# LarissaReames-NOAA/MPASSIT

Measured on AMD Instinct MI355X. Metric: interpolated 3-D fields/sec (nCells x nLev -> nx x ny), higher is better.
Workload: dtype f64

## Files before the change

### mpassit_amd/csrc/k_prims.hip

```cpp
#include "mpg_internal.h"

#define SCAN_NT 256
#define SCAN_IPT 16
#define SCAN_TILE (SCAN_NT * SCAN_IPT)

__global__ __launch_bounds__(SCAN_NT) void k_scan_block_sums(const int32_t *__restrict__ in, int64_t n, int32_t *__restrict__ bsum) {
  __shared__ int32_t ws[SCAN_NT / 64];
  const int64_t base = (int64_t)blockIdx.x * SCAN_TILE;
  int32_t v = 0;
#pragma unroll
  for (int k = 0; k < SCAN_IPT; ++k) {
    const int64_t i = base + (int64_t)k * SCAN_NT + threadIdx.x;
    if (i < n) v += in[i];
  }
  for (int o = 32; o > 0; o >>= 1) v += __shfl_down(v, o);
  if ((threadIdx.x & 63) == 0) ws[threadIdx.x >> 6] = v;
  __syncthreads();
  if (threadIdx.x == 0) bsum[blockIdx.x] = ws[0] + ws[1] + ws[2] + ws[3];
}

__device__ __forceinline__ int32_t block_excl_scan(int32_t v, int32_t *total) {
  __shared__ int32_t ws[SCAN_NT / 64 + 1];
  const int lane = threadIdx.x & 63, w = threadIdx.x >> 6;
  int32_t inc = v;
  for (int o = 1; o < 64; o <<= 1) {
    const int32_t t = __shfl_up(inc, o);
    if (lane >= o) inc += t;
  }
  __syncthreads();
  if (lane == 63) ws[w] = inc;
  __syncthreads();
  int32_t off = 0;
  for (int k = 0; k < w; ++k) off += ws[k];
  *total = ws[0] + ws[1] + ws[2] + ws[3];
  return off + inc - v;
}

__global__ __launch_bounds__(SCAN_NT) void k_scan_sums(int32_t *__restrict__ bsum, int64_t nb) {
  int32_t carry = 0;
  for (int64_t b0 = 0; b0 < nb; b0 += SCAN_NT) {
    const int64_t i = b0 + threadIdx.x;
    const int32_t v = i < nb ? bsum[i] : 0;
    int32_t total;
    const int32_t ex = block_excl_scan(v, &total);
    if (i < nb) bsum[i] = carry + ex;
    carry += total;
  }
}

__global__ __launch_bounds__(SCAN_NT) void k_scan_apply(const int32_t *in, int64_t n, const int32_t *__restrict__ boff, int32_t *out) {
  const int64_t base = (int64_t)blockIdx.x * SCAN_TILE + (int64_t)threadIdx.x * SCAN_IPT;
  int32_t v[SCAN_IPT];
  int32_t sum = 0;
#pragma unroll
  for (int k = 0; k < SCAN_IPT; ++k) {
    v[k] = base + k < n ? in[base + k] : 0;
    sum += v[k];
  }
  int32_t total;
  int32_t run = boff[blockIdx.x] + block_excl_scan(sum, &total);
#pragma unroll
  for (int k = 0; k < SCAN_IPT; ++k) {
    if (base + k < n) out[base + k] = run;
    run += v[k];
  }
}

int mpg_scan_excl_i32(const int32_t *in, int32_t *out, int64_t n, hipStream_t s) {
  if (n <= 0) return MPG_SUCCESS;
  const int64_t nb = (n + SCAN_TILE - 1) / SCAN_TILE;
  TmpBuf<int32_t> bsum;
  int rc;
  if ((rc = bsum.alloc((size_t)nb, s))) return rc;
  k_scan_block_sums<<<(unsigned)nb, SCAN_NT, 0, s>>>(in, n, bsum.p);
  k_scan_sums<<<1, SCAN_NT, 0, s>>>(bsum.p, nb);
  k_scan_apply<<<(unsigned)nb, SCAN_NT, 0, s>>>(in, n, bsum.p, out);
  MPG_HIP(hipGetLastError());
  return MPG_SUCCESS;
}

__global__ __launch_bounds__(256) void k_sum_i32_i64(const int32_t *__restrict__ in, int64_t n, unsigned long long *__restrict__ out) {
  __shared__ long long ws[4];
  long long v = 0;
  for (int64_t i = blockIdx.x * (int64_t)blockDim.x + threadIdx.x; i < n; i += (int64_t)gridDim.x * blockDim.x) v += in[i];
  for (int o = 32; o > 0; o >>= 1) v += __shfl_down(v, o);
  if ((threadIdx.x & 63) == 0) ws[threadIdx.x >> 6] = v;
  __syncthreads();
  if (threadIdx.x == 0) atomicAdd(out, (unsigned long long)(ws[0] + ws[1] + ws[2] + ws[3]));
}

int mpg_sum_i32_i64(const int32_t *in, int64_t n, long long *out_dev, hipStream_t s) {
  MPG_HIP(hipMemsetAsync(out_dev, 0, sizeof(long long), s));
  if (n > 0) k_sum_i32_i64<<<(unsigned)std::min<int64_t>((n + 255) / 256, 1024), 256, 0, s>>>(in, n, (unsigned long long *)out_dev);
  MPG_HIP(hipGetLastError());
  return MPG_SUCCESS;
}

const void *mpg_anchor_k_prims() { return (const void *)k_scan_apply; }
```

### mpassit_amd/csrc/k_store_conserve.hip

```cpp
#include <cstring>


#pragma clang fp contract(off)

#include "geom.h"
#include "mpg_internal.h"
#include "conserve_clip.h"

#define CONS_BUF (CONS_MAXV + 4)
#define CONS_STACK 64
static_assert(CONS_STACK >= WalkCap<PyrTree>::FILTER, "the stack holds the walk's proven bound (tree_walk.h): its guard is never taken");
#define CONS_QUEUE 2048

#define CAND_CAP 24
#define CONS_SPILL 256
#define CONS_BIGBOX 128
#define CONS_COOP_NT 64
template <int MODE>
__global__ __launch_bounds__(MODE == 3 ? 128 : CONS_COOP_NT) void k_conserve_raster(int64_t nCells, int maxEdges, const int32_t *__restrict__ voc,
                                                         const double *__restrict__ vx, const double *__restrict__ vy,
                                                         const double *__restrict__ vz, PyramidView pyr, int nx, int ny,
                                                         const double *__restrict__ qx, const double *__restrict__ qy,
                                                         const double *__restrict__ qz, const double *__restrict__ qarea,
                                                         const double *__restrict__ qsph, int32_t *__restrict__ cnt_src,
                                                         int32_t *__restrict__ tmp_dst, int32_t *__restrict__ ovf, int32_t *__restrict__ n_ovf,
                                                         uint8_t *__restrict__ flip, const int32_t *__restrict__ poff,
                                                         int32_t *__restrict__ pair_c, int32_t *__restrict__ pair_p, const float *__restrict__ vij,
                                                         float pad_coef, float pad_latlon, float e_max, int32_t *__restrict__ spill, int spill_cap) {
  constexpr bool COOP = MODE == 5 || MODE == 6;
  int64_t c = COOP ? (int64_t)ovf[blockIdx.x] : MODE == 7 ? (int64_t)pair_c[blockIdx.x] : blockIdx.x * (int64_t)blockDim.x + threadIdx.x;
  if (c >= nCells) return;
  if (MODE == 5 && cnt_src[c] != CAND_CAP + 1) return;
  if (MODE == 5 && n_ovf && threadIdx.x == 0) atomicAdd(n_ovf + 3, 1);
  if (spill && (int)blockIdx.x >= spill_cap && COOP) spill = nullptr;
  if (MODE == 6 && spill) {
    const int n = poff[c + 1] - poff[c];
    if (n <= CONS_SPILL) {
      if (n_ovf && threadIdx.x == 0) atomicAdd(n_ovf + 4, 1);
      for (int k = threadIdx.x; k < n; k += blockDim.x) {
        pair_c[poff[c] + k] = (int32_t)c;
        pair_p[poff[c] + k] = spill[(int64_t)blockIdx.x * CONS_SPILL + k];
      }
      return;
    }
  }
  int found = 0;
  dv3 poly[CONS_MAXV];
  int n = 0;
  for (int j = 0; j < maxEdges && n < CONS_MAXV; ++j) {
    int32_t v = voc[c * maxEdges + j];
    if (v > 0) poly[n++] = dv3{vx[v - 1], vy[v - 1], vz[v - 1]};
  }
  if (n < 3) return;
  double area = 0.0;
  for (int i = 1; i + 1 < n; ++i) area += sph_tri_area(poly[0], poly[i], poly[i + 1]);
  if (area == 0.0) return;
  if (MODE == 3 && flip) flip[c] = area < 0.0;
  if (area < 0.0)
    for (int i = 0; i < n / 2; ++i) {
      dv3 t = poly[i]; poly[i] = poly[n - 1 - i]; poly[n - 1 - i] = t;
    }
  double lo[3] = {2, 2, 2}, hi[3] = {-2, -2, -2}, e2 = 0.0;
  for (int i = 0; i < n; ++i) {
    lo[0] = fmin(lo[0], poly[i].x); hi[0] = fmax(hi[0], poly[i].x);
    lo[1] = fmin(lo[1], poly[i].y); hi[1] = fmax(hi[1], poly[i].y);
    lo[2] = fmin(lo[2], poly[i].z); hi[2] = fmax(hi[2], poly[i].z);
    dv3 d = poly[i] - poly[0];
    e2 = fmax(e2, dot3(d, d));
  }
  double pad = 2.0 * e2 + 1e-9;
#pragma unroll
  for (int k = 0; k < 3; ++k) { lo[k] -= pad; hi[k] += pad; }

  int nxc = nx + 1;
  auto candidate = [&](int i, int j) -> bool {
    const int64_t pc = (int64_t)j * nx + i;
    {
      const double4 sph = *reinterpret_cast<const double4 *>(qsph + 4 * pc);
      double sx = sph.x, sy = sph.y, sz = sph.z, r2 = sph.w;
      double ddx = fmax(fmax(lo[0] - sx, sx - hi[0]), 0.0), ddy = fmax(fmax(lo[1] - sy, sy - hi[1]), 0.0),
             ddz = fmax(fmax(lo[2] - sz, sz - hi[2]), 0.0);
      if (ddx * ddx + ddy * ddy + ddz * ddz > r2) return false;
    }
    int64_t k00 = (int64_t)j * nxc + i;
    dv3 q[4] = {dv3{qx[k00], qy[k00], qz[k00]}, dv3{qx[k00 + 1], qy[k00 + 1], qz[k00 + 1]},
                dv3{qx[k00 + nxc + 1], qy[k00 + nxc + 1], qz[k00 + nxc + 1]}, dv3{qx[k00 + nxc], qy[k00 + nxc], qz[k00 + nxc]}};
    double ql[3] = {2, 2, 2}, qh[3] = {-2, -2, -2}, qe2 = 0.0;
#pragma unroll
    for (int k = 0; k < 4; ++k) {
      ql[0] = fmin(ql[0], q[k].x); qh[0] = fmax(qh[0], q[k].x);
      ql[1] = fmin(ql[1], q[k].y); qh[1] = fmax(qh[1], q[k].y);
      ql[2] = fmin(ql[2], q[k].z); qh[2] = fmax(qh[2], q[k].z);
      dv3 d = q[k] - q[0];
      qe2 = fmax(qe2, dot3(d, d));
    }
    double qp = 2.0 * qe2 + 1e-9;
    if (ql[0] - qp > hi[0] || qh[0] + qp < lo[0] || ql[1] - qp > hi[1] || qh[1] + qp < lo[1] || ql[2] - qp > hi[2] || qh[2] + qp < lo[2]) return false;
    return fabs(qarea[pc]) > 0.0;
  };
  if ((MODE == 3 || MODE == 7) && vij) {
    float imin = 1e30f, imax = -1e30f, jmin = 1e30f, jmax = -1e30f;
    bool ok = true;
    for (int j = 0, k = 0; j < maxEdges && k < CONS_MAXV; ++j) {
      int32_t v = voc[c * maxEdges + j];
      if (v <= 0) continue;
      ++k;
      const float vi = vij[2 * (int64_t)(v - 1)], vj = vij[2 * (int64_t)(v - 1) + 1];
      ok = ok && vi == vi && vj == vj;
      imin = fminf(imin, vi); imax = fmaxf(imax, vi);
      jmin = fminf(jmin, vj); jmax = fmaxf(jmax, vj);
    }
    const float E = fmaxf(imax - imin, jmax - jmin);
    if (!ok) {
      const double *bx = pyr.box + 6 * pyr.off[pyr.nlev - 1];
      if (bx[0] > hi[0] || bx[3] < lo[0] || bx[1] > hi[1] || bx[4] < lo[1] || bx[2] > hi[2] || bx[5] < lo[2]) {
        cnt_src[c] = 0;
        return;
      }
      cnt_src[c] = CAND_CAP + 1;
      ovf[atomicAdd(n_ovf, 1)] = (int32_t)c;
      return;
    }
    if (E <= e_max) {
      const float pad = mpg_box_pad(E, pad_coef, pad_latlon, fmax(fabs(lo[2]), fabs(hi[2])));
      const int i0 = max((int)ceilf(imin - pad - 0.5f), 0), i1 = min((int)floorf(imax + pad + 0.5f), nx - 1);
      const int j0 = max((int)ceilf(jmin - pad - 0.5f), 0), j1 = min((int)floorf(jmax + pad + 0.5f), ny - 1);
      const int bw = max(i1 - i0 + 1, 0), bh = max(j1 - j0 + 1, 0);
      if (MODE == 3 && pair_c && bw * bh > CONS_BIGBOX) {
        const int qs = atomicAdd(n_ovf + 2, 1);
        if (qs < spill_cap) {
          pair_c[qs] = (int32_t)c;
          cnt_src[c] = CAND_CAP + 1;
          return;
        }
      }
      if (MODE == 7) {
        const int lane = (int)threadIdx.x, total = bw * bh;
        int slot = -1;
        bool complete = true;
        for (int base = 0; base < total && complete; base += 64) {
          const int q = base + lane;
          bool is = false;
          int32_t pc = 0;
          if (q < total) {
            const int i = i0 + q % bw, j = j0 + q / bw;
            is = candidate(i, j);
            pc = (int32_t)((int64_t)j * nx + i);
          }
          const unsigned long long mask = __ballot(is);
          const int nnew = __popcll(mask);
          if (nnew == 0) continue;
          const int pos = found + __popcll(mask & ((1ull << lane) - 1ull));
          if (found + nnew > CAND_CAP && slot < 0) {
            int sl = 0;
            if (lane == 0) {
              sl = atomicAdd(n_ovf, 1);
              ovf[sl] = (int32_t)c;
            }
            slot = __shfl(sl, 0);
            if (spill && slot < spill_cap) {
              __threadfence_block();
              for (int k = lane; k < min(found, CAND_CAP); k += 64) spill[(int64_t)slot * CONS_SPILL + k] = tmp_dst[c * CAND_CAP + k];
            } else {
              complete = false;
            }
          }
          if (is) {
            if (pos < CAND_CAP) tmp_dst[c * CAND_CAP + pos] = pc;
            if (slot >= 0 && complete && pos < CONS_SPILL) spill[(int64_t)slot * CONS_SPILL + pos] = pc;
          }
          found += nnew;
          if (slot >= 0 && found > CONS_SPILL) complete = false;
        }
        if (lane == 0) cnt_src[c] = (slot < 0 || complete) ? found : CAND_CAP + 1;
        return;
      }
      int slot = -1;
      bool complete = true;
      for (int j = j0; j <= j1; ++j)
        for (int i = i0; i <= i1; ++i) {
          if (!candidate(i, j)) continue;
          const int32_t pc = (int32_t)((int64_t)j * nx + i);
          if (found < CAND_CAP) {
            tmp_dst[c * CAND_CAP + found] = pc;
          } else {
            if (slot < 0) {
              slot = atomicAdd(n_ovf, 1);
              ovf[slot] = (int32_t)c;
              if (spill && slot < spill_cap)
                for (int k = 0; k < CAND_CAP; ++k) spill[(int64_t)slot * CONS_SPILL + k] = tmp_dst[c * CAND_CAP + k];
              else
                complete = false;
            }
            if (complete && found < CONS_SPILL) spill[(int64_t)slot * CONS_SPILL + found] = pc;
            else complete = false;
          }
          ++found;
          if (!complete) {
            j = j1;
            break;
          }
        }
      cnt_src[c] = (slot < 0 || complete) ? found : CAND_CAP + 1;
      return;
    }
  }
  if (MODE == 7) return;
  int stack[CONS_STACK];
  __shared__ int q_nodes[2][CONS_QUEUE];
  __shared__ int q_n[2], q_over, s_found;
  int seed_lev = pyr.nlev - 1, nseed = 1, cur = 0;
  if (COOP) {
    if (threadIdx.x == 0) { q_nodes[0][0] = 0; q_n[0] = 1; q_over = 0; s_found = 0; }
    __syncthreads();
    while (seed_lev > 1) {
      const int nq = q_n[cur];
      if (threadIdx.x == 0) q_n[cur ^ 1] = 0;
      __syncthreads();
      const int cnx = pyr.nx[seed_lev - 1], cny = pyr.ny[seed_lev - 1], pnx = pyr.nx[seed_lev];
      for (int k = threadIdx.x; k < nq; k += blockDim.x) {
        int node = q_nodes[cur][k], bi = node % pnx, bj = node / pnx;
        for (int ch = 0; ch < 4; ++ch) {
          int ci = 2 * bi + (ch & 1), cj = 2 * bj + (ch >> 1);
          if (ci >= cnx || cj >= cny) continue;
          const double *bx = pyr.box + 6 * (pyr.off[seed_lev - 1] + cj * cnx + ci);
          if (bx[0] > hi[0] || bx[3] < lo[0] || bx[1] > hi[1] || bx[4] < lo[1] || bx[2] > hi[2] || bx[5] < lo[2]) continue;
          int slot = atomicAdd(&q_n[cur ^ 1], 1);
          if (slot < CONS_QUEUE) q_nodes[cur ^ 1][slot] = cj * cnx + ci;
          else q_over = 1;
        }
      }
      __syncthreads();
      if (q_over) break;
      cur ^= 1;
      --seed_lev;
      __syncthreads();
    }
    nseed = q_n[cur];
  }
  for (int sk = COOP ? (int)threadIdx.x : 0; sk < nseed; sk += COOP ? (int)blockDim.x : 1) {
  const int seed = COOP ? q_nodes[cur][sk] : 0;
  int sp = 0;
  auto meets = [&](int lev_, int node_) -> bool {
    const double *bx = pyr.box + 6 * (pyr.off[lev_] + node_);
    return !(bx[0] > hi[0] || bx[3] < lo[0] || bx[1] > hi[1] || bx[4] < lo[1] || bx[2] > hi[2] || bx[5] < lo[2]);
  };
  int cur = (COOP || meets(seed_lev, seed)) ? ((seed_lev << 26) | seed) : -1;
  for (;;) {
    if (cur < 0) {
      if (sp == 0) break;
      cur = stack[--sp];
    }
    const int e = cur;
    cur = -1;
    int lev = e >> 26, node = e & ((1 << 26) - 1);
    int nxl = pyr.nx[lev];
    int bi = node % nxl, bj = node / nxl;
    if (lev == 0) {
      int i0 = bi * MPG_PYR_B0, j0 = bj * MPG_PYR_B0;
      int i1 = min(i0 + MPG_PYR_B0, nx), j1 = min(j0 + MPG_PYR_B0, ny);
      for (int j = j0; j < j1; ++j)
        for (int i = i0; i < i1; ++i) {
          if (!candidate(i, j)) continue;
          const int64_t p = (int64_t)j * nx + i;
          if (MODE == 3) {
            if (found == CAND_CAP) {
              cnt_src[c] = CAND_CAP + 1;
              ovf[atomicAdd(n_ovf, 1)] = (int32_t)c;
              return;
            }
            tmp_dst[c * CAND_CAP + found] = (int32_t)p;
            ++found;
          } else if (MODE == 5) {
            const int slot = atomicAdd(&s_found, 1);
            if (spill && slot < CONS_SPILL) spill[(int64_t)blockIdx.x * CONS_SPILL + slot] = (int32_t)p;
          } else {
            const int slot = atomicAdd(&s_found, 1);
            pair_c[poff[c] + slot] = (int32_t)c;
            pair_p[poff[c] + slot] = (int32_t)p;
          }
        }
    } else {
      int cnx = pyr.nx[lev - 1], cny = pyr.ny[lev - 1];
      bool go[4];
#pragma unroll
      for (int ch = 0; ch < 4; ++ch) {
        int ci = 2 * bi + (ch & 1), cj = 2 * bj + (ch >> 1);
        go[ch] = ci < cnx && cj < cny && meets(lev - 1, cj * cnx + ci);
      }
#pragma unroll
      for (int ch = 0; ch < 4; ++ch)
        if (go[ch]) {
          const int child = ((lev - 1) << 26) | ((2 * bj + (ch >> 1)) * cnx + 2 * bi + (ch & 1));
          if (cur < 0) cur = child;
          else if (sp < CONS_STACK) stack[sp++] = child;
        }
    }
  }
  }
  if (MODE == 3) cnt_src[c] = found;
  if (MODE == 5) {
    __syncthreads();
    if (threadIdx.x == 0) cnt_src[c] = s_found;
  }
}

__global__ __launch_bounds__(256) void k_cell_areas(int nx, int ny, const double *__restrict__ qx, const double *__restrict__ qy,
                                                    const double *__restrict__ qz, double *__restrict__ qarea,
                                                    double *__restrict__ qsph ) {
  int64_t p = blockIdx.x * (int64_t)blockDim.x + threadIdx.x;
  if (p >= (int64_t)nx * ny) return;
  int i = (int)(p % nx), j = (int)(p / nx), nxc = nx + 1;
  int64_t k00 = (int64_t)j * nxc + i;
  dv3 q0 = dv3{qx[k00], qy[k00], qz[k00]}, q1 = dv3{qx[k00 + 1], qy[k00 + 1], qz[k00 + 1]},
      q2 = dv3{qx[k00 + nxc + 1], qy[k00 + nxc + 1], qz[k00 + nxc + 1]}, q3 = dv3{qx[k00 + nxc], qy[k00 + nxc], qz[k00 + nxc]};
  qarea[p] = sph_tri_area(q0, q1, q2) + sph_tri_area(q0, q2, q3);
  dv3 cen = (q0 + q1) + (q2 + q3);
  double nn = sqrt(dot3(cen, cen));
  cen = nn > 0.0 ? cen * (1.0 / nn) : q0;
  double r2 = 0.0;
  dv3 d = q0 - cen; r2 = fmax(r2, dot3(d, d));
  d = q1 - cen; r2 = fmax(r2, dot3(d, d));
  d = q2 - cen; r2 = fmax(r2, dot3(d, d));
  d = q3 - cen; r2 = fmax(r2, dot3(d, d));
  *reinterpret_cast<double4 *>(qsph + 4 * p) = double4{cen.x, cen.y, cen.z, r2 * (1.0 + 1e-9) + 1e-18};
}

__global__ __launch_bounds__(256) void k_max_valence(int64_t nCells, int maxEdges, const int32_t *__restrict__ voc, int32_t *__restrict__ out) {
  __shared__ int smax;
  if (threadIdx.x == 0) smax = 0;
  __syncthreads();
  int mx = 0;
  for (int64_t c = blockIdx.x * (int64_t)blockDim.x + threadIdx.x; c < nCells; c += (int64_t)gridDim.x * blockDim.x) {
    int n = 0;
    for (int j = 0; j < maxEdges; ++j) n += voc[c * maxEdges + j] > 0;
    mx = max(mx, n);
  }
  atomicMax(&smax, mx);
  __syncthreads();
  if (threadIdx.x == 0) atomicMax(out, smax);
}

int mpg_k_mesh_max_valence(mpg_mesh_s *m, hipStream_t s) {
  if (m->max_valence >= 0) return MPG_SUCCESS;
  int rc;
  TmpBuf<int32_t> mv;
  if ((rc = mv.alloc(1, s))) return rc;
  MPG_HIP(hipMemsetAsync(mv.p, 0, sizeof(int32_t), s));
  const int64_t nC = m->cwn;
  int32_t hv = 0;
  if (nC > 0) k_max_valence<<<(unsigned)std::min<int64_t>((nC + 255) / 256, 2048), 256, 0, s>>>(nC, m->maxEdges, m->voc.p, mv.p);
  MPG_HIP(hipGetLastError());
  MPG_HIP(hipMemcpyAsync(&hv, mv.p, sizeof(int32_t), hipMemcpyDeviceToHost, s));
  MPG_HIP(hipStreamSynchronize(s));
  m->max_valence = hv;
  return MPG_SUCCESS;
}

__global__ __launch_bounds__(256) void k_csr_sort_rows(int64_t P, const int32_t *__restrict__ rowptr, int32_t *__restrict__ col,
                                                       double *__restrict__ val) {
  int64_t p = blockIdx.x * (int64_t)blockDim.x + threadIdx.x;
  if (p >= P) return;
  int b = rowptr[p], e = rowptr[p + 1];
  for (int i = b + 1; i < e; ++i) {
    int32_t kc = col[i];
    double kv = val[i];
    int j = i - 1;
    while (j >= b && col[j] > kc) {
      col[j + 1] = col[j];
      val[j + 1] = val[j];
      --j;
    }
    col[j + 1] = kc;
    val[j + 1] = kv;
  }
}

__global__ __launch_bounds__(256) void k_conserve_clamp_counts(int64_t nCells, const int32_t *__restrict__ cnt_src, int32_t *__restrict__ npair) {
  int64_t c = blockIdx.x * (int64_t)blockDim.x + threadIdx.x;
  if (c > nCells) return;
  int n = c < nCells ? cnt_src[c] : 0;
  npair[c] = n;
}
__global__ __launch_bounds__(256) void k_conserve_fill_pairs(int64_t nCells, const int32_t *__restrict__ npair, const int32_t *__restrict__ poff,
                                                             const int32_t *__restrict__ tmp_dst, int32_t *__restrict__ pair_c,
                                                             int32_t *__restrict__ pair_p) {
  int64_t c = blockIdx.x * (int64_t)blockDim.x + threadIdx.x;
  if (c >= nCells) return;
  const int n = npair[c], o = poff[c];
  if (n > CAND_CAP) return;
  for (int e = 0; e < n; ++e) {
    pair_c[o + e] = (int32_t)c;
    pair_p[o + e] = tmp_dst[c * CAND_CAP + e];
  }
}

template <bool RAW>
__global__ __launch_bounds__(CLIP_NT) void k_conserve_clip_pairs(int64_t npairs, const int32_t *__restrict__ pair_c, const int32_t *__restrict__ pair_p,
                                                                 int maxEdges, const int32_t *__restrict__ voc, const double *__restrict__ vx,
                                                                 const double *__restrict__ vy, const double *__restrict__ vz,
                                                                 const uint8_t *__restrict__ flip, int nx, const double *__restrict__ qx,
                                                                 const double *__restrict__ qy, const double *__restrict__ qz,
                                                                 const double *__restrict__ qarea, int cb, double *__restrict__ pair_val,
                                                                 int32_t *__restrict__ count, int32_t *__restrict__ truncated) {
  extern __shared__ double clip_lds[];
  const int64_t t = blockIdx.x * (int64_t)CLIP_NT + threadIdx.x;
  if (t >= npairs) return;
  const LdsPoly L{clip_lds + threadIdx.x, cb};
  const int64_t c = pair_c[t], p = pair_p[t];
  int32_t vid[CONS_MAXV];
#pragma unroll
  for (int k = 0; k < CONS_MAXV; ++k) vid[k] = k < maxEdges ? voc[c * maxEdges + k] : 0;
  const bool rev = flip[c] != 0;
  int ntot = 0, vsafe = 0;
#pragma unroll
  for (int k = 0; k < CONS_MAXV; ++k) {
    if (vid[k] > 0) {
      ++ntot;
      if (vsafe == 0) vsafe = vid[k];
    }
  }
  int n = 0;
  if (vsafe > 0) {
    dv3 vc[CONS_MAXV];
#pragma unroll
    for (int k = 0; k < CONS_MAXV; ++k) {
      const int64_t v = (vid[k] > 0 ? vid[k] : vsafe) - 1;
      vc[k] = dv3{vx[v], vy[v], vz[v]};
    }
#pragma unroll
    for (int k = 0; k < CONS_MAXV; ++k)
      if (vid[k] > 0) {
        L.set(0, rev ? ntot - 1 - n : n, vc[k]);
        ++n;
      }
  }
  const int i = (int)(p % nx), j = (int)(p / nx), nxc = nx + 1;
  const int64_t k00 = (int64_t)j * nxc + i;
  dv3 q[4] = {dv3{qx[k00], qy[k00], qz[k00]}, dv3{qx[k00 + 1], qy[k00 + 1], qz[k00 + 1]},
              dv3{qx[k00 + nxc + 1], qy[k00 + nxc + 1], qz[k00 + nxc + 1]}, dv3{qx[k00 + nxc], qy[k00 + nxc], qz[k00 + nxc]}};
  double aq = qarea[p];
  if (aq < 0.0) { dv3 tq = q[1]; q[1] = q[3]; q[3] = tq; aq = -aq; }
  double ar = 0.0;
  int trunc = 0;
  if (aq > 0.0) {
    const int cur = 0;
    for (int e = 0; e < 4 && n >= 3; ++e) {
      const dv3 qa = e == 0 ? q[0] : e == 1 ? q[1] : e == 2 ? q[2] : q[3];
      const dv3 qb = e == 0 ? q[1] : e == 1 ? q[2] : e == 2 ? q[3] : q[0];
      dv3 side = qb - qa;
      if (dot3(side, side) < 1e-24) continue;
      n = clip_halfspace_lds(n, L, cross3(qa, side), cb, &trunc);
    }
    if (n >= 3) {
      double sa = 0.0;
      const dv3 v0 = L.get(cur, 0);
      for (int k = 1; k + 1 < n; ++k) sa += sph_tri_area(v0, L.get(cur, k), L.get(cur, k + 1));
      ar = sa > 0.0 ? sa : 0.0;
    }
  }
  if constexpr (RAW) {
    pair_val[t] = ar;
  } else {
    double ratio = 0.0;
    if (ar > 1e-14 * aq) {
      ratio = ar / aq;
      atomicAdd(&count[p], 1);
    }
    pair_val[t] = ratio;
  }
  if (trunc) atomicOr(truncated, 1);
}
__global__ __launch_bounds__(256) void k_conserve_scatter_pairs(int64_t npairs, const int32_t *__restrict__ pair_c, const int32_t *__restrict__ pair_p,
                                                                const double *__restrict__ pair_val, const int32_t *__restrict__ rowptr,
                                                                int32_t *__restrict__ cursor, int32_t *__restrict__ col, double *__restrict__ val,
                                                                int32_t cell0) {
  int64_t t = blockIdx.x * (int64_t)blockDim.x + threadIdx.x;
  if (t >= npairs) return;
  const double r = pair_val[t];
  if (!(r > 0.0)) return;
  const int32_t p = pair_p[t];
  const int slot = atomicAdd(&cursor[p], 1);
  col[rowptr[p] + slot] = pair_c[t] + cell0;
  val[rowptr[p] + slot] = r;
}

struct ConsPairs {
  TmpBuf<int32_t> count, cnt_src, tmp_dst, ovf, n_ovf, npair, poff, pair_c, pair_p, spill, bigq, truncated;
  TmpBuf<double> qarea, qsph, pair_val;
  TmpBuf<uint8_t> flip;
  TmpBuf<float> vij;
  int32_t npairs = 0, novf = 0, nbig = 0;
  int cb = 0;
};
static int conserve_pairs(mpg_mesh_s *m, mpg_grid_s *g, mpg_handle_s *h, hipStream_t s, bool raw, ConsPairs &X) {
  int rc;
  PointSet &cor = g->pts[MPG_STAGGERLOC_CORNER];
  const int nx = g->nx, ny = g->ny;
  const int64_t P = (int64_t)nx * ny;
  TmpBuf<int32_t> &count = X.count, &cnt_src = X.cnt_src, &tmp_dst = X.tmp_dst, &ovf = X.ovf, &n_ovf = X.n_ovf, &npair = X.npair, &poff = X.poff,
                  &pair_c = X.pair_c, &pair_p = X.pair_p;
  TmpBuf<double> &qarea = X.qarea, &qsph = X.qsph, &pair_val = X.pair_val;
  TmpBuf<uint8_t> &flip = X.flip;
  const int64_t nC = m->cwn;
  const double *vx = m->vx_g(), *vy = m->vy_g(), *vz = m->vz_g();
  if ((!raw && (rc = count.alloc((size_t)P + 1, s))) || (rc = qarea.alloc((size_t)P, s)) || (rc = qsph.alloc(4 * (size_t)P, s)) ||
      (rc = cnt_src.alloc((size_t)nC, s)) || (rc = tmp_dst.alloc((size_t)nC * CAND_CAP, s)) || (rc = ovf.alloc((size_t)nC, s)) || (rc = n_ovf.alloc(5, s)) ||
      (rc = npair.alloc((size_t)nC + 1, s)) || (rc = poff.alloc((size_t)nC + 1, s)) || (rc = flip.alloc((size_t)nC, s)))
    return rc;
  MPG_HIP(hipMemsetAsync(n_ovf.p, 0, 5 * sizeof(int32_t), s));
  MPG_HIP(hipMemsetAsync(cnt_src.p, 0, sizeof(int32_t) * (size_t)nC, s));
  MPG_HIP(hipMemsetAsync(flip.p, 0, (size_t)nC, s));
  if (!raw) MPG_HIP(hipMemsetAsync(count.p, 0, sizeof(int32_t) * (P + 1), s));
  unsigned nb = (unsigned)((nC + 127) / 128);
  PyramidView pv = mpg_pyr_view(g->cellpyr);
  TmpBuf<float> &vij = X.vij;
  const float *vijp = nullptr;
  if (mpg_grid_has_inverse(g, MPG_STAGGERLOC_CORNER) && mpg_store_boxes() && m->vwn > 0) {
    if ((rc = vij.alloc(2 * (size_t)m->vwn, s))) return rc;
    if ((rc = mpg_k_points_ij(g, m->vwn, m->vert.x.p, m->vert.y.p, m->vert.z.p, vij.p, s))) return rc;
    vijp = vij.p - 2 * m->vw0;
    h->store_path = 1;
  }
  k_cell_areas<<<(unsigned)((P + 255) / 256), 256, 0, s>>>(nx, ny, cor.x.p, cor.y.p, cor.z.p, qarea.p, qsph.p);
  const int spill_cap = (int)std::min<int64_t>(nC, 1 << 16);
  TmpBuf<int32_t> &spill = X.spill, &bigq = X.bigq;
  if ((rc = spill.alloc((size_t)spill_cap * CONS_SPILL, s)) || (rc = bigq.alloc((size_t)spill_cap, s))) return rc;
  k_conserve_raster<3><<<nb, 128, 0, s>>>(nC, m->maxEdges, m->voc.p, vx, vy, vz, pv, nx, ny, cor.x.p, cor.y.p, cor.z.p,
                                        qarea.p, qsph.p, cnt_src.p, tmp_dst.p, ovf.p, n_ovf.p, flip.p, nullptr, vijp ? bigq.p : nullptr, nullptr, vijp,
                                        (float)mpg_grid_box_pad_coef(g), (float)mpg_grid_box_pad_latlon(g), (float)mpg_grid_box_emax(g), spill.p, spill_cap);
  if (m->max_valence < 0) k_max_valence<<<(unsigned)std::min<int64_t>((nC + 255) / 256, 2048), 256, 0, s>>>(nC, m->maxEdges, m->voc.p, n_ovf.p + 1);
  MPG_HIP(hipGetLastError());
  int32_t &novf = X.novf, hv[3] = {0, 0, 0};
  MPG_HIP(hipMemcpyAsync(hv, n_ovf.p, 3 * sizeof(int32_t), hipMemcpyDeviceToHost, s));
  MPG_HIP(hipStreamSynchronize(s));
  novf = hv[0];
  if (m->max_valence < 0) m->max_valence = hv[1];
  if (hv[2] > 0) {
    k_conserve_raster<7><<<(unsigned)std::min(hv[2], spill_cap), 64, 0, s>>>(nC, m->maxEdges, m->voc.p, vx, vy, vz, pv, nx, ny, cor.x.p, cor.y.p, cor.z.p,
                                                                            qarea.p, qsph.p, cnt_src.p, tmp_dst.p, ovf.p, n_ovf.p, nullptr, nullptr, bigq.p, nullptr,
                                                                            vijp, (float)mpg_grid_box_pad_coef(g), (float)mpg_grid_box_pad_latlon(g),
                                                                            (float)mpg_grid_box_emax(g), spill.p, spill_cap);
    MPG_HIP(hipGetLastError());
    MPG_HIP(hipMemcpyAsync(&novf, n_ovf.p, sizeof(int32_t), hipMemcpyDeviceToHost, s));
    MPG_HIP(hipStreamSynchronize(s));
  }
  const unsigned coop_nt = CONS_COOP_NT;
  if (novf > 0)
    k_conserve_raster<5><<<(unsigned)novf, coop_nt, 0, s>>>(nC, m->maxEdges, m->voc.p, vx, vy, vz, pv, nx, ny, cor.x.p,
                                                       cor.y.p, cor.z.p, qarea.p, qsph.p, cnt_src.p, nullptr, ovf.p, n_ovf.p, nullptr, nullptr,
                                                       nullptr, nullptr, nullptr, 0.f, 0.f, 0.f, spill.p, spill_cap);
  k_conserve_clamp_counts<<<(unsigned)((nC + 256) / 256), 256, 0, s>>>(nC, cnt_src.p, npair.p);
  if ((rc = mpg_scan_excl_i32(npair.p, poff.p, nC + 1, s))) return rc;
  int32_t &npairs = X.npairs;
  long long total = 0;
  {
    TmpBuf<long long> tot;
    if ((rc = tot.alloc(1, s))) return rc;
    if ((rc = mpg_sum_i32_i64(npair.p, nC, tot.p, s))) return rc;
    MPG_HIP(hipMemcpyAsync(&npairs, poff.p + nC, sizeof(int32_t), hipMemcpyDeviceToHost, s));
    MPG_HIP(hipMemcpyAsync(&total, tot.p, sizeof(total), hipMemcpyDeviceToHost, s));
    MPG_HIP(hipStreamSynchronize(s));
    if (npairs < 0 || total != (long long)npairs) {
      mpg_set_error("conservative RegridStore: %lld candidate pairs exceed 2^31", total);
      return MPG_ERR_OVERFLOW;
    }
  }
  if ((rc = pair_c.alloc((size_t)npairs + 1, s)) || (rc = pair_p.alloc((size_t)npairs + 1, s)) || (rc = pair_val.alloc((size_t)npairs + 1, s))) return rc;
  k_conserve_fill_pairs<<<(unsigned)((nC + 255) / 256), 256, 0, s>>>(nC, npair.p, poff.p, tmp_dst.p, pair_c.p, pair_p.p);
  if (novf > 0)
    k_conserve_raster<6><<<(unsigned)novf, coop_nt, 0, s>>>(nC, m->maxEdges, m->voc.p, vx, vy, vz, pv, nx, ny, cor.x.p,
                                                       cor.y.p, cor.z.p, qarea.p, qsph.p, nullptr, nullptr, ovf.p, n_ovf.p, nullptr, poff.p,
                                                       pair_c.p, pair_p.p, nullptr, 0.f, 0.f, 0.f, spill.p, spill_cap);
  MPG_HIP(hipGetLastError());
  const int nv = std::max(3, std::min(m->max_valence, m->maxEdges));
  const int cb = X.cb = nv + 4 < CONS_BUF ? nv + 4 : CONS_BUF;
  const size_t clip_lds_bytes = sizeof(double) * cb * 3 * CLIP_NT;
  auto clip = raw ? k_conserve_clip_pairs<true> : k_conserve_clip_pairs<false>;
  if (clip_lds_bytes > 48 * 1024) MPG_HIP(hipFuncSetAttribute((const void *)clip, hipFuncAttributeMaxDynamicSharedMemorySize, (int)clip_lds_bytes));
  TmpBuf<int32_t> &truncated = X.truncated;
  if ((rc = truncated.alloc(1, s))) return rc;
  MPG_HIP(hipMemsetAsync(truncated.p, 0, sizeof(int32_t), s));
  if (npairs > 0)
    clip<<<(unsigned)(((int64_t)npairs + CLIP_NT - 1) / CLIP_NT), CLIP_NT, clip_lds_bytes, s>>>(
        npairs, pair_c.p, pair_p.p, m->maxEdges, m->voc.p, vx, vy, vz, flip.p, nx, cor.x.p, cor.y.p, cor.z.p, qarea.p, cb,
        pair_val.p, raw ? nullptr : count.p, truncated.p);
  MPG_HIP(hipGetLastError());
  X.nbig = std::min(hv[2], spill_cap);
  return MPG_SUCCESS;
}

int mpg_k_store_conserve(mpg_mesh_s *m, mpg_grid_s *g, mpg_handle_s *h, hipStream_t s) {
  int rc;
  PointSet &cor = g->pts[MPG_STAGGERLOC_CORNER];
  int nx = g->nx, ny = g->ny;
  int64_t P = (int64_t)nx * ny;
  if (cor.n != (int64_t)(nx + 1) * (ny + 1)) {
    mpg_set_error("conservative RegridStore needs CORNER-stagger coordinates on the destination grid");
    return MPG_ERR_INVALID_ARG;
  }
  if (m->maxEdges > CONS_MAXV) {
    mpg_set_error("conservative RegridStore: maxEdges %d > %d", m->maxEdges, CONS_MAXV);
    return MPG_ERR_UNSUPPORTED;
  }
  if (!g->cellpyr.built && (rc = mpg_k_build_cell_pyramid(cor, nx, ny, g->cellpyr, s))) return rc;
  if ((rc = mpg_walk_check<PyrTree>((int64_t)g->cellpyr.nx[0] * g->cellpyr.ny[0], "conservative RegridStore"))) return rc;
  h->kind = MPG_KIND_CSR;
  h->nnz_per_row = 0;
  h->n_src = m->nCells;
  h->n_dst = P;
  h->nx_dst = nx;
  h->ny_dst = ny;
  const int64_t nC = m->cwn;
  if (nC == 0) {
    if ((rc = h->rowptr.alloc((size_t)P + 1)) || (rc = h->col.alloc(1)) || (rc = h->val.alloc(1))) return rc;
    MPG_HIP(hipMemsetAsync(h->rowptr.p, 0, sizeof(int32_t) * (P + 1), s));
    MPG_HIP(hipStreamSynchronize(s));
    h->nnz = 0;
    return MPG_SUCCESS;
  }
  ConsPairs X;
  if ((rc = h->rowptr.alloc((size_t)P + 1)) || (rc = conserve_pairs(m, g, h, s, false, X))) return rc;
  TmpBuf<int32_t> &count = X.count, &n_ovf = X.n_ovf, &truncated = X.truncated, &pair_c = X.pair_c, &pair_p = X.pair_p;
  TmpBuf<double> &pair_val = X.pair_val;
  const int32_t npairs = X.npairs, novf = X.novf;
  const int cb = X.cb;
  if ((rc = mpg_scan_excl_i32(count.p, h->rowptr.p, P + 1, s))) return rc;
  int32_t nnz = 0, was_truncated = 0, hs[5] = {0, 0, 0, 0, 0};
  MPG_HIP(hipMemcpyAsync(hs, n_ovf.p, sizeof(hs), hipMemcpyDeviceToHost, s));
  MPG_HIP(hipMemcpyAsync(&nnz, h->rowptr.p + P, sizeof(int32_t), hipMemcpyDeviceToHost, s));
  MPG_HIP(hipMemcpyAsync(&was_truncated, truncated.p, sizeof(int32_t), hipMemcpyDeviceToHost, s));
  MPG_HIP(hipStreamSynchronize(s));
  if (was_truncated) {
    mpg_set_error("conservative RegridStore: a clipped polygon outgrew its %d vertex slots (a non-convex source cell?)", cb);
    return MPG_ERR_OVERFLOW;
  }
  if (nnz < 0) {
    mpg_set_error("conservative weight matrix exceeds 2^31 entries");
    return MPG_ERR_OVERFLOW;
  }
  h->nnz = nnz;
  h->store_stats[1] = npairs; h->store_stats[2] = novf; h->store_stats[3] = X.nbig; h->store_stats[4] = hs[3];
  h->store_stats[5] = hs[4]; h->store_stats[6] = cb;
  if ((rc = h->col.alloc((size_t)nnz + 1)) || (rc = h->val.alloc((size_t)nnz + 1))) return rc;
  MPG_HIP(hipMemsetAsync(count.p, 0, sizeof(int32_t) * (P + 1), s));
  if (npairs > 0)
    k_conserve_scatter_pairs<<<(unsigned)(((int64_t)npairs + 255) / 256), 256, 0, s>>>(npairs, pair_c.p, pair_p.p, pair_val.p, h->rowptr.p, count.p,
                                                                                      h->col.p, h->val.p, (int32_t)m->cw0);
  k_csr_sort_rows<<<(unsigned)((P + 255) / 256), 256, 0, s>>>(P, h->rowptr.p, h->col.p, h->val.p);
  MPG_HIP(hipGetLastError());
  MPG_HIP(hipStreamSynchronize(s));
  return MPG_SUCCESS;
}

__global__ __launch_bounds__(256) void k_conserve_tm_count(int64_t nCells, int maxEdges, const int32_t *__restrict__ voc, const double *__restrict__ vx,
                                                           const double *__restrict__ vy, const double *__restrict__ vz,
                                                           const int32_t *__restrict__ poff, const double *__restrict__ pair_val,
                                                           double *__restrict__ carea, int32_t *__restrict__ cnt) {
  const int64_t c = blockIdx.x * (int64_t)blockDim.x + threadIdx.x;
  if (c > nCells) return;
  if (c == nCells) {
    cnt[c] = 0;
    return;
  }
  const double a = cell_fan_area(c, maxEdges, voc, vx, vy, vz);
  carea[c] = a;
  int n = 0;
  if (a > 0.0)
    for (int t = poff[c]; t < poff[c + 1]; ++t) n += pair_val[t] > 1e-14 * a;
  cnt[c] = n;
}
__global__ __launch_bounds__(256) void k_conserve_tm_rows(int64_t nCells, const int32_t *__restrict__ poff, const int32_t *__restrict__ pair_p,
                                                          const double *__restrict__ pair_val, const double *__restrict__ carea,
                                                          const int32_t *__restrict__ rowptr, int norm_type, int32_t *__restrict__ col,
                                                          double *__restrict__ val, double *__restrict__ frac) {
  const int64_t c = blockIdx.x * (int64_t)blockDim.x + threadIdx.x;
  if (c >= nCells) return;
  const double a = carea[c];
  const int b = rowptr[c], e = rowptr[c + 1];
  if (e == b) {
    frac[c] = 0.0;
    return;
  }
  int n = 0;
  for (int t = poff[c]; t < poff[c + 1]; ++t) {
    const double I = pair_val[t];
    if (!(I > 1e-14 * a)) continue;
    const int32_t g = pair_p[t];
    int j = b + n - 1;
    while (j >= b && col[j] > g) {
      col[j + 1] = col[j];
      val[j + 1] = val[j];
      --j;
    }
    col[j + 1] = g;
    val[j + 1] = I;
    ++n;
  }
  double sum = 0.0;
  for (int q = b; q < e; ++q) sum += val[q];
  frac[c] = sum / a;
  const double d = norm_type == MPG_NORM_FRACAREA ? sum : a;
  for (int q = b; q < e; ++q) val[q] = val[q] / d;
}

int mpg_k_conserve_rows(mpg_mesh_s *m, const int32_t *poff, const int32_t *pair_col, const double *pair_val, const int32_t *truncated, int cb,
                        int norm_type, const char *who, mpg_handle_s *h, hipStream_t s, const int32_t *extra_dev, int32_t *extra_host, int nextra) {
  int rc;
  const int64_t nC = m->nCells;
  TmpBuf<double> carea;
  TmpBuf<int32_t> cnt;
  if ((rc = carea.alloc((size_t)nC, s)) || (rc = cnt.alloc((size_t)nC + 1, s))) return rc;
  const double *vx = m->vx_g(), *vy = m->vy_g(), *vz = m->vz_g();
  k_conserve_tm_count<<<(unsigned)((nC + 256) / 256), 256, 0, s>>>(nC, m->maxEdges, m->voc.p, vx, vy, vz, poff, pair_val, carea.p, cnt.p);
  MPG_HIP(hipGetLastError());
  if ((rc = mpg_scan_excl_i32(cnt.p, h->rowptr.p, nC + 1, s))) return rc;
  int32_t nnz = 0, was_truncated = 0;
  if (nextra > 0) MPG_HIP(hipMemcpyAsync(extra_host, extra_dev, sizeof(int32_t) * (size_t)nextra, hipMemcpyDeviceToHost, s));
  MPG_HIP(hipMemcpyAsync(&nnz, h->rowptr.p + nC, sizeof(int32_t), hipMemcpyDeviceToHost, s));
  MPG_HIP(hipMemcpyAsync(&was_truncated, truncated, sizeof(int32_t), hipMemcpyDeviceToHost, s));
  MPG_HIP(hipStreamSynchronize(s));
  if (was_truncated) {
    mpg_set_error("%s: a clipped polygon outgrew its %d vertex slots (a non-convex mesh cell?)", who, cb);
    return MPG_ERR_OVERFLOW;
  }
  if (nnz < 0) {
    mpg_set_error("%s: the weight matrix exceeds 2^31 entries", who);
    return MPG_ERR_OVERFLOW;
  }
  h->nnz = nnz;
  if ((rc = h->col.alloc((size_t)nnz + 1)) || (rc = h->val.alloc((size_t)nnz + 1))) return rc;
  k_conserve_tm_rows<<<(unsigned)((nC + 255) / 256), 256, 0, s>>>(nC, poff, pair_col, pair_val, carea.p, h->rowptr.p, norm_type, h->col.p, h->val.p,
                                                                  h->dst_frac.p);
  MPG_HIP(hipGetLastError());
  MPG_HIP(hipStreamSynchronize(s));
  return MPG_SUCCESS;
}

int mpg_k_store_conserve_to_mesh(mpg_grid_s *g, mpg_mesh_s *m, int norm_type, mpg_handle_s *h, hipStream_t s) {
  int rc;
  PointSet &cor = g->pts[MPG_STAGGERLOC_CORNER];
  const int nx = g->nx, ny = g->ny;
  if (cor.n != (int64_t)(nx + 1) * (ny + 1)) {
    mpg_set_error("mpg_regrid_store_conserve_to_mesh: a conservative Store needs CORNER-stagger coordinates on the source grid");
    return MPG_ERR_INVALID_ARG;
  }
  if (m->maxEdges > CONS_MAXV) {
    mpg_set_error("mpg_regrid_store_conserve_to_mesh: maxEdges %d > %d", m->maxEdges, CONS_MAXV);
    return MPG_ERR_UNSUPPORTED;
  }
  if (!g->cellpyr.built && (rc = mpg_k_build_cell_pyramid(cor, nx, ny, g->cellpyr, s))) return rc;
  if ((rc = mpg_walk_check<PyrTree>((int64_t)g->cellpyr.nx[0] * g->cellpyr.ny[0], "mpg_regrid_store_conserve_to_mesh"))) return rc;
  const int64_t nC = m->nCells;
  h->kind = MPG_KIND_CSR;
  h->nnz_per_row = 0;
  h->n_src = (int64_t)nx * ny;
  h->n_dst = nC;
  h->nx_dst = (int)nC;
  h->ny_dst = 1;
  if ((rc = h->rowptr.alloc((size_t)nC + 1)) || (rc = h->dst_frac.alloc((size_t)std::max<int64_t>(nC, 1)))) return rc;
  if (nC == 0) {
    MPG_HIP(hipMemsetAsync(h->rowptr.p, 0, sizeof(int32_t), s));
    MPG_HIP(hipStreamSynchronize(s));
    if ((rc = h->col.alloc(1)) || (rc = h->val.alloc(1))) return rc;
    h->nnz = 0;
    return MPG_SUCCESS;
  }
  ConsPairs X;
  if ((rc = conserve_pairs(m, g, h, s, true, X))) return rc;
  int32_t hs[5] = {0, 0, 0, 0, 0};
  if ((rc = mpg_k_conserve_rows(m, X.poff.p, X.pair_p.p, X.pair_val.p, X.truncated.p, X.cb, norm_type, "mpg_regrid_store_conserve_to_mesh", h, s, X.n_ovf.p, hs, 5)))
    return rc;
  h->store_stats[1] = X.npairs; h->store_stats[2] = X.novf; h->store_stats[3] = X.nbig; h->store_stats[4] = hs[3];
  h->store_stats[5] = hs[4]; h->store_stats[6] = X.cb;
  return MPG_SUCCESS;
}

const void *mpg_anchor_k_store_conserve() { return (const void *)k_cell_areas; }
```

### mpassit_amd/csrc/k_store_conserve_mesh.hip

```cpp
#pragma clang fp contract(off)
#include <math.h>

#include <algorithm>

#include "geom.h"
#include "mpg_internal.h"
#include "conserve_clip.h"

#define CM_STACK 96

static_assert(CM_STACK >= WalkCap<BvhTree>::FILTER, "the stack holds the walk's proven bound (tree_walk.h): its guard is never taken");
__device__ __forceinline__ bool cell_box(int64_t c, int maxEdges, const int32_t *__restrict__ voc, const double *__restrict__ vx,
                                         const double *__restrict__ vy, const double *__restrict__ vz, double *lo, double *hi) {
  lo[0] = lo[1] = lo[2] = 2.0;
  hi[0] = hi[1] = hi[2] = -2.0;
  dv3 first = dv3{0, 0, 0};
  double e2 = 0.0;
  int n = 0;
  for (int j = 0; j < maxEdges && n < CONS_MAXV; ++j) {
    const int32_t v = voc[c * maxEdges + j];
    if (v <= 0) continue;
    const dv3 x = dv3{vx[v - 1], vy[v - 1], vz[v - 1]};
    if (n == 0) first = x;
    lo[0] = fmin(lo[0], x.x); hi[0] = fmax(hi[0], x.x);
    lo[1] = fmin(lo[1], x.y); hi[1] = fmax(hi[1], x.y);
    lo[2] = fmin(lo[2], x.z); hi[2] = fmax(hi[2], x.z);
    const dv3 d = x - first;
    e2 = fmax(e2, dot3(d, d));
    ++n;
  }
  if (n < 3) {
    lo[0] = lo[1] = lo[2] = 2.0;
    hi[0] = hi[1] = hi[2] = -2.0;
    return false;
  }
  const double pad = 2.0 * e2 + 1e-9;
#pragma unroll
  for (int k = 0; k < 3; ++k) {
    lo[k] -= pad;
    hi[k] += pad;
  }
  return true;
}

__global__ __launch_bounds__(256) void k_cell_orient(int64_t nC, int maxEdges, const int32_t *__restrict__ voc, const double *__restrict__ vx,
                                                     const double *__restrict__ vy, const double *__restrict__ vz, uint8_t *__restrict__ orient) {
  const int64_t c = blockIdx.x * (int64_t)blockDim.x + threadIdx.x;
  if (c >= nC) return;
  dv3 first = dv3{0, 0, 0}, prev = first;
  int n = 0;
  double area = 0.0;
  for (int j = 0; j < maxEdges && n < CONS_MAXV; ++j) {
    const int32_t v = voc[c * maxEdges + j];
    if (v <= 0) continue;
    const dv3 x = dv3{vx[v - 1], vy[v - 1], vz[v - 1]};
    if (n == 0) first = x;
    else if (n >= 2) area += sph_tri_area(first, prev, x);
    prev = x;
    ++n;
  }
  orient[c] = (n < 3 || area == 0.0) ? 2 : (area < 0.0 ? 1 : 0);
}

__global__ __launch_bounds__(256) void k_cbvh_cellbox(int64_t n, const int32_t *__restrict__ sid, int maxEdges, const int32_t *__restrict__ voc,
                                                      const double *__restrict__ vx, const double *__restrict__ vy,
                                                      const double *__restrict__ vz, double *__restrict__ cellbox) {
  const int64_t i = blockIdx.x * (int64_t)blockDim.x + threadIdx.x;
  if (i >= n) return;
  double lo[3], hi[3];
  cell_box(sid[i], maxEdges, voc, vx, vy, vz, lo, hi);
  double *o = cellbox + 6 * i;
  o[0] = lo[0]; o[1] = lo[1]; o[2] = lo[2]; o[3] = hi[0]; o[4] = hi[1]; o[5] = hi[2];
}

static int build_cell_bvh(mpg_mesh_s *m, hipStream_t s) {
  CellBvh &b = m->cbvh;
  if (b.built) return MPG_SUCCESS;
  int rc;
  const int64_t n = m->nCells;
  if ((rc = b.cellbox.alloc(6 * (size_t)n))) return rc;
  rc = mpg_bvh_build(
      b, n, "mpg_regrid_store_conserve_mesh",
      [&](unsigned long long *key, int32_t *id) { return mpg_k_morton(n, m->cell.x.p, m->cell.y.p, m->cell.z.p, key, id, 0, s); },
      [&]() {
        k_cbvh_cellbox<<<(unsigned)((n + 255) / 256), 256, 0, s>>>(n, b.sorted_id.p, m->maxEdges, m->voc.p, m->vert.x.p, m->vert.y.p, m->vert.z.p,
                                                                   b.cellbox.p);
        static_assert(MPG_BVH_LEAF == MPG_BVH_FAN, "a leaf's box is the hull of its cells' boxes as an upper node's is of its children's");
        return mpg_k_bvh_up(n, b.nnodes[0], b.cellbox.p, b.box.p, s);
      },
      s, true);
  if (rc) b.free();
  return rc;
}

template <bool FILL>
__global__ __launch_bounds__(256) void k_cm_candidates(int64_t nD, int maxEdges, const int32_t *__restrict__ voc, const double *__restrict__ vx,
                                                       const double *__restrict__ vy, const double *__restrict__ vz,
                                                       const uint8_t *__restrict__ orient_d, const uint8_t *__restrict__ orient_s, CellBvhView b,
                                                       int32_t *__restrict__ cnt, const int32_t *__restrict__ poff, int32_t *__restrict__ pair_d,
                                                       int32_t *__restrict__ pair_s, int32_t *__restrict__ overflow) {
  const int64_t d = blockIdx.x * (int64_t)blockDim.x + threadIdx.x;
  if (d > nD) return;
  if (d == nD) {
    if (!FILL) cnt[d] = 0;
    return;
  }
  double lo[3], hi[3];
  int found = 0;
  const bool poly = orient_d[d] != 2 && cell_box(d, maxEdges, voc, vx, vy, vz, lo, hi);
  if (poly && b.n > 0) {
    const int32_t o = FILL ? poff[d] : 0, oe = FILL ? poff[d + 1] : 0;
    auto meets = [&](const double *bx) -> bool {
      return !(bx[0] > hi[0] || bx[3] < lo[0] || bx[1] > hi[1] || bx[4] < lo[1] || bx[2] > hi[2] || bx[5] < lo[2]);
    };
    int stack[CM_STACK];
    int sp = 0;
    const int top = b.nlev - 1;
    int cur = meets(b.box + 6 * b.off[top]) ? (top << 27) : -1;
    for (;;) {
      if (cur < 0) {
        if (sp == 0) break;
        cur = stack[--sp];
      }
      const int e = cur;
      cur = -1;
      const int lev = e >> 27;
      const int64_t node = e & ((1 << 27) - 1);
      if (lev == 0) {
        const int64_t i1 = min(b.n, (node + 1) * MPG_BVH_LEAF);
        for (int64_t i = node * MPG_BVH_LEAF; i < i1; ++i) {
          if (!meets(b.cellbox + 6 * i)) continue;
          const int32_t sc = b.sid[i];
          if (orient_s[sc] == 2) continue;
          if (FILL) {
            if (o + found < oe) {
              pair_d[o + found] = (int32_t)d;
              pair_s[o + found] = sc;
            }
          }
          ++found;
        }
        continue;
      }
      const int64_t c0 = node * MPG_BVH_FAN, c1 = min(b.nnodes[lev - 1], c0 + MPG_BVH_FAN);
      for (int64_t c = c0; c < c1; ++c) {
        if (!meets(b.box + 6 * (b.off[lev - 1] + c))) continue;
        const int enc = ((lev - 1) << 27) | (int)c;
        if (cur < 0) cur = enc;
        else if (sp < CM_STACK) stack[sp++] = enc;
        else atomicOr(overflow, 1);
      }
    }
  }
  if (!FILL) cnt[d] = found;
}

__global__ __launch_bounds__(CLIP_NT) void k_cm_clip_pairs(int64_t npairs, const int32_t *__restrict__ pair_d, const int32_t *__restrict__ pair_s,
                                                           int me_s, const int32_t *__restrict__ voc_s, const double *__restrict__ sx,
                                                           const double *__restrict__ sy, const double *__restrict__ sz,
                                                           const uint8_t *__restrict__ orient_s, int me_d, const int32_t *__restrict__ voc_d,
                                                           const double *__restrict__ dx, const double *__restrict__ dy,
                                                           const double *__restrict__ dz, const uint8_t *__restrict__ orient_d, int cb,
                                                           double *__restrict__ pair_val, int32_t *__restrict__ truncated) {
  extern __shared__ double cm_clip_lds[];
  const int64_t t = blockIdx.x * (int64_t)CLIP_NT + threadIdx.x;
  if (t >= npairs) return;
  const LdsPoly L{cm_clip_lds + threadIdx.x, cb};
  const int64_t d = pair_d[t], c = pair_s[t];
  int32_t vid_s[CONS_MAXV], vid_d[CONS_MAXV];
#pragma unroll
  for (int k = 0; k < CONS_MAXV; ++k) {
    vid_s[k] = k < me_s ? voc_s[c * me_s + k] : 0;
    vid_d[k] = k < me_d ? voc_d[d * me_d + k] : 0;
  }
  const bool rev_s = orient_s[c] == 1, rev_d = orient_d[d] == 1;
  int ns_tot = 0, nd_tot = 0, safe_s = 0, safe_d = 0;
#pragma unroll
  for (int k = 0; k < CONS_MAXV; ++k) {
    if (vid_s[k] > 0) {
      ++ns_tot;
      if (safe_s == 0) safe_s = vid_s[k];
    }
    if (vid_d[k] > 0) {
      ++nd_tot;
      if (safe_d == 0) safe_d = vid_d[k];
    }
  }
  double ar = 0.0;
  int trunc = 0;
  if (safe_s > 0 && safe_d > 0 && ns_tot <= cb && nd_tot <= cb) {
    dv3 vs[CONS_MAXV], vd[CONS_MAXV];
#pragma unroll
    for (int k = 0; k < CONS_MAXV; ++k) {
      const int64_t a = (vid_s[k] > 0 ? vid_s[k] : safe_s) - 1, b = (vid_d[k] > 0 ? vid_d[k] : safe_d) - 1;
      vs[k] = dv3{sx[a], sy[a], sz[a]};
      vd[k] = dv3{dx[b], dy[b], dz[b]};
    }
    int nd = 0;
#pragma unroll
    for (int k = 0; k < CONS_MAXV; ++k)
      if (vid_d[k] > 0) {
        L.set(0, rev_d ? nd_tot - 1 - nd : nd, vd[k]);
        ++nd;
      }
    dv3 q[CONS_MAXV];
#pragma unroll
    for (int k = 0; k < CONS_MAXV; ++k) q[k] = k < nd ? L.get(0, k) : dv3{0, 0, 0};
    int n = 0;
#pragma unroll
    for (int k = 0; k < CONS_MAXV; ++k)
      if (vid_s[k] > 0) {
        L.set(0, rev_s ? ns_tot - 1 - n : n, vs[k]);
        ++n;
      }
    const dv3 qfirst = q[0];
    for (int e = 0; e < nd && n >= 3; ++e) {
      const dv3 qa = q[0], qb = e + 1 == nd ? qfirst : q[1];
#pragma unroll
      for (int k = 0; k + 1 < CONS_MAXV; ++k) q[k] = q[k + 1];
      const dv3 side = qb - qa;
      if (dot3(side, side) < 1e-24) continue;
      n = clip_halfspace_lds(n, L, cross3(qa, side), cb, &trunc);
    }
    if (n >= 3) {
      double sa = 0.0;
      const dv3 v0 = L.get(0, 0);
      for (int k = 1; k + 1 < n; ++k) sa += sph_tri_area(v0, L.get(0, k), L.get(0, k + 1));
      ar = sa > 0.0 ? sa : 0.0;
    }
  }
  pair_val[t] = ar;
  if (trunc) atomicOr(truncated, 1);
}

int mpg_k_store_conserve_mesh(mpg_mesh_s *src, mpg_mesh_s *dst, int norm_type, mpg_handle_s *h, hipStream_t s) {
  int rc;
  if (src->maxEdges > CONS_MAXV || dst->maxEdges > CONS_MAXV) {
    mpg_set_error("mpg_regrid_store_conserve_mesh: maxEdges %d > %d", std::max(src->maxEdges, dst->maxEdges), CONS_MAXV);
    return MPG_ERR_UNSUPPORTED;
  }
  const int64_t nS = src->nCells, nD = dst->nCells;
  h->kind = MPG_KIND_CSR;
  h->nnz_per_row = 0;
  h->n_src = nS;
  h->n_dst = nD;
  h->nx_dst = (int)nD;
  h->ny_dst = 1;
  h->store_path = 0;
  if ((rc = h->rowptr.alloc((size_t)nD + 1)) || (rc = h->dst_frac.alloc((size_t)std::max<int64_t>(nD, 1)))) return rc;
  if (nD == 0 || nS == 0) {
    MPG_HIP(hipMemsetAsync(h->rowptr.p, 0, sizeof(int32_t) * (size_t)(nD + 1), s));
    if (nD > 0) MPG_HIP(hipMemsetAsync(h->dst_frac.p, 0, sizeof(double) * (size_t)nD, s));
    MPG_HIP(hipStreamSynchronize(s));
    if ((rc = h->col.alloc(1)) || (rc = h->val.alloc(1))) return rc;
    h->nnz = 0;
    return MPG_SUCCESS;
  }
  if ((rc = mpg_k_mesh_max_valence(src, s)) || (rc = mpg_k_mesh_max_valence(dst, s))) return rc;
  const bool had = src->cbvh.built;
  if ((rc = build_cell_bvh(src, s))) return rc;
  const CellBvh &b = src->cbvh;
  CellBvhView v;
  mpg_bvh_view(b, v);
  v.cellbox = b.cellbox.p;
  const double *sx = src->vert.x.p, *sy = src->vert.y.p, *sz = src->vert.z.p, *dx = dst->vert.x.p, *dy = dst->vert.y.p, *dz = dst->vert.z.p;
  TmpBuf<uint8_t> orient_s, orient_d;
  if ((rc = orient_s.alloc((size_t)nS, s))) return rc;
  k_cell_orient<<<(unsigned)((nS + 255) / 256), 256, 0, s>>>(nS, src->maxEdges, src->voc.p, sx, sy, sz, orient_s.p);
  const uint8_t *od = orient_s.p;
  if (dst != src) {
    if ((rc = orient_d.alloc((size_t)nD, s))) return rc;
    k_cell_orient<<<(unsigned)((nD + 255) / 256), 256, 0, s>>>(nD, dst->maxEdges, dst->voc.p, dx, dy, dz, orient_d.p);
    od = orient_d.p;
  }
  MPG_HIP(hipGetLastError());
  TmpBuf<int32_t> cnt, poff, ovf, pair_d, pair_s, truncated;
  TmpBuf<double> pair_val;
  if ((rc = cnt.alloc((size_t)nD + 1, s)) || (rc = poff.alloc((size_t)nD + 1, s)) || (rc = ovf.alloc(1, s)) || (rc = truncated.alloc(1, s))) return rc;
  MPG_HIP(hipMemsetAsync(ovf.p, 0, sizeof(int32_t), s));
  MPG_HIP(hipMemsetAsync(truncated.p, 0, sizeof(int32_t), s));
  const unsigned nbd = (unsigned)((nD + 256) / 256);
  k_cm_candidates<false><<<nbd, 256, 0, s>>>(nD, dst->maxEdges, dst->voc.p, dx, dy, dz, od, orient_s.p, v, cnt.p, nullptr, nullptr, nullptr, ovf.p);
  MPG_HIP(hipGetLastError());
  if ((rc = mpg_scan_excl_i32(cnt.p, poff.p, nD + 1, s))) return rc;
  int32_t npairs = 0, h_ovf = 0;
  long long total = 0;
  {
    TmpBuf<long long> tot;
    if ((rc = tot.alloc(1, s))) return rc;
    if ((rc = mpg_sum_i32_i64(cnt.p, nD, tot.p, s))) return rc;
    MPG_HIP(hipMemcpyAsync(&npairs, poff.p + nD, sizeof(int32_t), hipMemcpyDeviceToHost, s));
    MPG_HIP(hipMemcpyAsync(&total, tot.p, sizeof(total), hipMemcpyDeviceToHost, s));
    MPG_HIP(hipMemcpyAsync(&h_ovf, ovf.p, sizeof(int32_t), hipMemcpyDeviceToHost, s));
    MPG_HIP(hipStreamSynchronize(s));
    if (h_ovf) {
      mpg_set_error("mpg_regrid_store_conserve_mesh: the traversal stack of the candidate search overflowed");
      return MPG_ERR_OVERFLOW;
    }
    if (npairs < 0 || total != (long long)npairs) {
      mpg_set_error("mpg_regrid_store_conserve_mesh: %lld candidate pairs exceed 2^31", total);
      return MPG_ERR_OVERFLOW;
    }
  }
  if ((rc = pair_d.alloc((size_t)npairs + 1, s)) || (rc = pair_s.alloc((size_t)npairs + 1, s)) || (rc = pair_val.alloc((size_t)npairs + 1, s))) return rc;
  k_cm_candidates<true><<<nbd, 256, 0, s>>>(nD, dst->maxEdges, dst->voc.p, dx, dy, dz, od, orient_s.p, v, nullptr, poff.p, pair_d.p, pair_s.p, ovf.p);
  MPG_HIP(hipGetLastError());
  const int nvs = std::max(3, std::min(src->max_valence, src->maxEdges)), nvd = std::max(3, std::min(dst->max_valence, dst->maxEdges));
  const int cb = nvs + nvd;
  const size_t clip_lds_bytes = sizeof(double) * cb * 3 * CLIP_NT;
  if (clip_lds_bytes > 48 * 1024)
    MPG_HIP(hipFuncSetAttribute((const void *)k_cm_clip_pairs, hipFuncAttributeMaxDynamicSharedMemorySize, (int)clip_lds_bytes));
  if (npairs > 0)
    k_cm_clip_pairs<<<(unsigned)(((int64_t)npairs + CLIP_NT - 1) / CLIP_NT), CLIP_NT, clip_lds_bytes, s>>>(
        npairs, pair_d.p, pair_s.p, src->maxEdges, src->voc.p, sx, sy, sz, orient_s.p, dst->maxEdges, dst->voc.p, dx, dy, dz, od, cb, pair_val.p,
        truncated.p);
  MPG_HIP(hipGetLastError());
  if ((rc = mpg_k_conserve_rows(dst, poff.p, pair_s.p, pair_val.p, truncated.p, cb, norm_type, "mpg_regrid_store_conserve_mesh", h, s))) return rc;
  h->store_stats[1] = npairs;
  h->store_stats[2] = 0;
  h->store_stats[3] = had ? 0 : (int64_t)(b.build_ms * 1e3f);
  h->store_stats[6] = cb;
  return MPG_SUCCESS;
}

const void *mpg_anchor_k_store_conserve_mesh() { return (const void *)k_cell_orient; }
```

### mpassit_amd/csrc/mpg_internal.h

```cpp
#pragma once
#include <hip/hip_runtime.h>
#include <stdint.h>
#include <functional>
#include <map>
#include <string>
#include <tuple>
#include <vector>

#include "../../include/mpassit_amd.h"
#include "tree_walk.h"

#ifndef MPG_TILE_ALIGN
#define MPG_TILE_ALIGN 32
#endif
static inline __host__ __device__ int mpg_tile_align(int nx, int dmax = 8) {
  for (int a = MPG_TILE_ALIGN; a >= 8; a >>= 1) {
    int d = nx % a;
    d = d < a - d ? d : a - d;
    if (d <= dmax) return a;
  }
  return MPG_TILE_ALIGN >= 8 ? 8 : 1;
}
static inline __host__ __device__ int mpg_tile_shift(int j, int nx, int align = -1) {
  if (align < 0) align = mpg_tile_align(nx);
  return align > 1 ? (int)(((long long)j * nx) % align) : 0;
}
static inline int mpg_tile_ntx(int nx, int txu, int align = -1) {
  if (align < 0) align = mpg_tile_align(nx);
  return (nx + (align > 1 && nx % align ? align - 1 : 0) + txu - 1) / txu;
}

#define MPG_WAVE 64

void mpg_set_error(const char *fmt, ...);
bool mpg_is_initialized();
hipStream_t mpg_setup_stream();

#define MPG_HIP(call)                                                                         \
  do {                                                                                        \
    hipError_t e_ = (call);                                                                   \
    if (e_ != hipSuccess) {                                                                   \
      mpg_set_error("%s failed: %s (%s:%d)", #call, hipGetErrorString(e_), __FILE__, __LINE__); \
      return MPG_ERR_HIP;                                                                     \
    }                                                                                         \
  } while (0)

#define MPG_CHECK_INIT()                                                               \
  do {                                                                                 \
    if (!mpg_is_initialized()) {                                                       \
      mpg_set_error("mpg_init has not been called (or no HIP device): no CPU fallback"); \
      return MPG_ERR_NOT_INITIALIZED;                                                  \
    }                                                                                  \
  } while (0)

#define MPG_ARG(cond, msg)         \
  do {                             \
    if (!(cond)) {                 \
      mpg_set_error("%s", msg);    \
      return MPG_ERR_INVALID_ARG;  \
    }                              \
  } while (0)

void mpg_release_caches();

template <typename T>
struct DevBuf {
  T *p = nullptr;
  size_t n = 0;
  int alloc(size_t count) {
    n = count;
    if (count == 0) return MPG_SUCCESS;
    if (hipMalloc((void **)&p, count * sizeof(T)) != hipSuccess) {
      (void)hipGetLastError();
      mpg_release_caches();
      MPG_HIP(hipMalloc((void **)&p, count * sizeof(T)));
    }
    return MPG_SUCCESS;
  }
  void free() {
    if (p) (void)hipFree(p);
    p = nullptr;
    n = 0;
  }
};

void *mpg_pool_get(size_t bytes, hipStream_t s);
void mpg_pool_put(void *p, size_t bytes, hipStream_t s);
void mpg_pool_release();
template <typename T>
struct TmpBuf : DevBuf<T> {
  bool pooled = false;
  hipStream_t pool_stream = nullptr;
  size_t pool_bytes = 0;
  TmpBuf() = default;
  TmpBuf(const TmpBuf &) = delete;
  TmpBuf &operator=(const TmpBuf &) = delete;
  ~TmpBuf() { free(); }
  using DevBuf<T>::alloc;
  int alloc(size_t count, hipStream_t s) {
    free();
    this->n = count;
    if (count == 0) return MPG_SUCCESS;
    pool_bytes = count * sizeof(T);
    this->p = (T *)mpg_pool_get(pool_bytes, s);
    if (!this->p) return MPG_ERR_HIP;
    pooled = true;
    pool_stream = s;
    return MPG_SUCCESS;
  }
  void free() {
    if (pooled && this->p) {
      mpg_pool_put(this->p, pool_bytes, pool_stream);
      this->p = nullptr;
      this->n = 0;
    } else {
      DevBuf<T>::free();
    }
    pooled = false;
  }
};

struct PointSet {
  int64_t n = 0;
  DevBuf<double> x, y, z;
  int alloc(int64_t count) {
    n = count;
    int rc;
    if ((rc = x.alloc(count))) return rc;
    if ((rc = y.alloc(count))) return rc;
    return z.alloc(count);
  }
  void free() { x.free(); y.free(); z.free(); n = 0; }
};

struct Pyramid {
  int nlev = 0;
  int nx[MPG_PYR_MAXLEV], ny[MPG_PYR_MAXLEV];
  int64_t off[MPG_PYR_MAXLEV + 1];
  DevBuf<double> box;
  bool built = false;
  void free() { box.free(); built = false; nlev = 0; }
};

struct Bvh {
  int64_t n = 0;
  DevBuf<int32_t> sorted_id;
  int nlev = 0;
  int64_t nnodes[MPG_BVH_MAXLEV];
  int64_t off[MPG_BVH_MAXLEV + 1];
  DevBuf<double> box;
  bool built = false;
  float build_ms = 0.f;
  void free() { sorted_id.free(); box.free(); built = false; }
};
typedef Bvh TriBvh;
struct SiteBvh : Bvh {
  PointSet sorted;
  void free() { sorted.free(); Bvh::free(); }
};
struct SiteBvhView : BvhView {
  const double *sx, *sy, *sz;
};
struct CellBvh : Bvh {
  DevBuf<double> cellbox;
  void free() { cellbox.free(); Bvh::free(); }
};
struct CellBvhView : BvhView {
  const double *cellbox;
};

struct mpg_handle_s;
struct mpg_grid_s;
typedef std::tuple<void *, int, void *, int, int> HandleKey;

struct mpg_mesh_s {
  int64_t nCells = 0, nVertices = 0;
  int maxEdges = 0;
  PointSet cell, vert;
  PointSet edge;
  DevBuf<double> angle_edge;
  DevBuf<int32_t> voc;
  DevBuf<int32_t> tri;
  int64_t nTriValid = 0;
  DevBuf<int32_t> fan;
  int fan_origin = 0;
  SiteBvh bvh;
  TriBvh tbvh;
  CellBvh cbvh;
  int64_t win_first[2] = {0, 0}, win_count[2] = {-1, -1};
  int64_t cw0 = 0, cwn = 0, vw0 = 0, vwn = 0;
  mpg_grid_s *geo_grid = nullptr;
  bool geo_grid_gone = false;
  double geo_margin = 0.0;
  int max_valence = -1;
  bool bvh_whole = true;
  const int32_t *voc_g() const { return voc.p - cw0 * maxEdges; }
  const double *vx_g() const { return vert.x.p - vw0; }
  const double *vy_g() const { return vert.y.p - vw0; }
  const double *vz_g() const { return vert.z.p - vw0; }
};

struct ProjDev {
  int code;
  double hemi, truelat1, truelat2, stdlon, cone, polei, polej, rebydx, lat1, lon1, knowni, knownj, latinc, loninc;
  double rsw, dlon;
  int nxmin, nxmax;
};

struct mpg_grid_s {
  int nx = 0, ny = 0, periodic = 0;
  PointSet pts[4];
  int snx[4], sny[4];
  Pyramid pyr[4];
  Pyramid cellpyr;
  Pyramid quadpyr[4];
  Pyramid wrappyr;
  int end_pole[2] = {0, 0};
  bool from_proj = false;
  int proj_code = 0;
  ProjDev proj;
  bool has_inverse = false;
  bool inverse_ok[4] = {true, true, true, true};
  int proj_row0 = 0;
  DevBuf<double> lon[4], lat[4];
  DevBuf<double> mapfac[3];
  DevBuf<double> cosa, sina;
};

enum { MPG_KIND_FIXED = 0, MPG_KIND_CSR = 1 };
struct mpg_handle_s {
  int kind = MPG_KIND_FIXED;
  int method = 0;
  int nnz_per_row = 0;
  int64_t n_src = 0, n_dst = 0;
  int nx_dst = 0, ny_dst = 0;
  DevBuf<int32_t> idx;
  DevBuf<double> w;
  DevBuf<int32_t> rowptr;
  DevBuf<int32_t> col;
  DevBuf<double> val;
  int64_t nnz = 0;
  DevBuf<double> dst_frac;
  int refcount = 1;
  bool cached = false;
  uint64_t parked_at = 0;
  HandleKey key;
  float store_ms = 0.f;
  int64_t store_stats[8] = {0, 0, 0, 0, 0, 0, 0, 0};
  int store_path = 0;
  bool localized = false;
  bool src_range_valid = false;
  int64_t src_range_first = 0, src_range_end = 0;
  int64_t n_pole = 0;
  int pole_len = 0;
  DevBuf<int32_t> pole_dst, pole_src0;
  DevBuf<double> pole_w;
  int ut_rpt = 0, ut_max = 0;
  int ut_align = MPG_TILE_ALIGN;
  int64_t ut_total = 0;
  int64_t ut_lines = 0, ut2_lines = 0;
  int lf_choice = 0;
  int cf_choice = 0;
  int cf_for = -99;
  float lf_reuse = 0.f;
  DevBuf<int32_t> ut_cnt, ut_cells;
  int ut_stride = 0, ut2_stride = 0;
  DevBuf<uint16_t> lidx;
  DevBuf<int32_t> ut_order, ut2_order;
  int ut_cls_off[7] = {0, 0, 0, 0, 0, 0, 0}, ut2_cls_off[7] = {0, 0, 0, 0, 0, 0, 0};
  int ut2_rpt = 0, ut2_max = 0, ut2_align = MPG_TILE_ALIGN;
  int64_t ut2_total = 0;
  DevBuf<int32_t> ut2_cnt, ut2_cells;
  DevBuf<uint16_t> lidx2;
  bool tr_built = false;
  DevBuf<int32_t> tr_ptr, tr_row, tr_long;
  DevBuf<double> tr_w;
  int64_t tr_nnz = 0, tr_nref = 0, tr_max = 0;
  int tr_nlong = 0;
  float tr_build_ms = 0.f;
  void free_transpose() {
    tr_ptr.free(); tr_row.free(); tr_long.free(); tr_w.free();
    tr_built = false;
    tr_nnz = tr_nref = tr_max = 0;
    tr_nlong = 0;
  }
  void free_tile_lists() {
    ut_cnt.free(); ut_cells.free(); lidx.free(); ut2_cnt.free(); ut2_cells.free(); lidx2.free(); ut_order.free(); ut2_order.free();
    ut_rpt = ut2_rpt = 0;
    free_transpose();
  }
};

void mpg_lfu_set_min_reuse_x10(int v);
int mpg_field_band(int kernel_default);
void mpg_set_field_band(int v);
void mpg_lfu_set_npf(int v);
void mpg_set_staged_store(int v);
void mpg_set_lf_rows_store(int v);
void mpg_set_staged_lds_pad_kb(int v);
int mpg_staged_lds_pad_kb();
bool mpg_handle_is_windowed(const mpg_handle_s *h);
void mpg_cache_detach(mpg_handle_s *h);
void mpg_hostpipe_release();
void mpg_fileio_release();

int mpg_k_mesh_coords(int64_t n, const double *lon_rad, const double *lat_rad, PointSet &out, hipStream_t s);
int mpg_k_grid_coords(int64_t n, const double *lon_deg, const double *lat_deg, PointSet &out, hipStream_t s);
int mpg_k_target_grid(const mpg_proj *proj, mpg_grid_s *g, hipStream_t s);
bool mpg_grid_has_inverse(const mpg_grid_s *g, int stagger = MPG_STAGGERLOC_CENTER);
int mpg_k_attach_proj(mpg_grid_s *g, const mpg_proj *proj, int row0, hipStream_t s);
#define MPG_LATLON_BOX_LIMIT 85.0
int mpg_k_points_ij(const mpg_grid_s *g, int64_t n, const double *x, const double *y, const double *z, float *ij, hipStream_t s, double latlon_limit = MPG_LATLON_BOX_LIMIT,
                    bool unwrap_i = false);
double mpg_grid_box_pad_latlon(const mpg_grid_s *g);
double mpg_grid_box_pad_coef(const mpg_grid_s *g);
double mpg_grid_box_emax(const mpg_grid_s *g);
double mpg_grid_min_index_chord(const mpg_grid_s *g, double lat_lo, double lat_hi, double margin);
int mpg_k_dual_triangles(mpg_mesh_s *m, hipStream_t s);
int mpg_k_tri_scatter(mpg_mesh_s *m, int32_t *cnt, hipStream_t s);
int mpg_k_tri_canon(mpg_mesh_s *m, const int32_t *cnt, hipStream_t s);
int mpg_k_mesh_window(mpg_mesh_s *m, mpg_grid_s *g, const double *latVertex, const double *lonVertex, const int32_t *verticesOnCell, hipStream_t s);
int mpg_k_voc_check(const int32_t *voc_dev, int64_t nent, int64_t nV, const char *who, hipStream_t s);
int mpg_k_mesh_coords_dev(int64_t n, const double *lon_rad_dev, const double *lat_rad_dev, double *x, double *y, double *z, unsigned long long *bad_dev,
                          hipStream_t s);
int mpg_k_build_pyramid(const PointSet &pts, int nx, int ny, Pyramid &pyr, hipStream_t s);
int mpg_k_build_cell_pyramid(const PointSet &corner, int nx, int ny, Pyramid &pyr, hipStream_t s);
int mpg_k_build_wrap_pyramid(const PointSet &pts, int nx, int ny, Pyramid &pyr, hipStream_t s);
PyramidView mpg_pyr_view(const Pyramid &p);
template <class Tree>
static inline int mpg_walk_check(int64_t leaves, const char *who) {
  if (walk_fits<Tree>(leaves)) return MPG_SUCCESS;
  mpg_set_error("%s: %lld tree leaves are too many for the walk (2^%d at most)", who, (long long)leaves, Tree::SHIFT);
  return MPG_ERR_OVERFLOW;
}
int mpg_k_store_bilinear_mesh(mpg_mesh_s *m, mpg_grid_s *g, int stagger, int meshloc, mpg_handle_s *h, hipStream_t s);
int mpg_k_store_nearest(mpg_mesh_s *m, mpg_grid_s *g, int stagger, mpg_handle_s *h, hipStream_t s);
int mpg_k_store_conserve(mpg_mesh_s *m, mpg_grid_s *g, mpg_handle_s *h, hipStream_t s);
int mpg_k_store_grid_bilinear(mpg_grid_s *g, int dst_stagger, mpg_handle_s *h, hipStream_t s);
int mpg_k_build_bvh(mpg_mesh_s *m, hipStream_t s, bool whole = true);
int mpg_zero_planes(void *dst, size_t esz, int64_t P, int64_t nplanes, int64_t ld, hipStream_t s);
#define MPG_TAB_MAX 32
struct FieldTab {
  const void *src[MPG_TAB_MAX];
  void *dst[MPG_TAB_MAX];
  double off[MPG_TAB_MAX];
  int n;
  __host__ __device__ FieldTab() : src{}, dst{}, off{}, n(0) {}
};
template <typename TS>
__device__ __forceinline__ const TS *mpg_field_src(const FieldTab &t, const TS *src, int f, int64_t slab) {
  return t.n ? (const TS *)t.src[f] : src + (int64_t)f * slab;
}
template <typename TD>
__device__ __forceinline__ TD *mpg_field_dst(const FieldTab &t, TD *dst, int f, int64_t slab) {
  return t.n ? (TD *)t.dst[f] : dst + (int64_t)f * slab;
}
__device__ __forceinline__ double mpg_field_off(const FieldTab &t, int f, double offset) { return t.n ? t.off[f] : offset; }
int mpg_k_apply_typed(mpg_handle_s *h, const void *src, int src_type, int layout, int nlev, int nfields, void *dst, int dst_type,
                      double scale, double offset, hipStream_t s, const FieldTab &tab = FieldTab(), int64_t ld = 0, bool epi = true);
enum { MPG_LF_ROWS = 0, MPG_LF_STAGED = 1, MPG_LF_ROWTILES = 2 };
#ifndef MPG_LF_STAGED_DEFAULT
#define MPG_LF_STAGED_DEFAULT MPG_LF_STAGED
#endif
#define MPG_STAGE_MIN_LEVELS 8
int mpg_cfu_num_variants();
int mpg_k_apply3_cfu(mpg_handle_s *h, int variant, const void *src, int src_f32, int nlev, int nfields, void *dst, int dst_f32, bool epi,
                     double scale, double offset, hipStream_t s, const FieldTab &tab = FieldTab(), int64_t ld = 0);
int mpg_k_apply3_lfu_typed(mpg_handle_s *h, const void *src, int src_type, int nlev, int nfields, void *dst, int dst_type, bool epi, double scale,
                           double offset, hipStream_t s, const FieldTab &tab = FieldTab(), int64_t ld = 0);
int mpg_a3_staged();
int mpg_lf_variant();
int mpg_lfu_build_shape(mpg_handle_s *h, int txu, int tyu, hipStream_t s);
int mpg_cfu_fits(mpg_handle_s *h, int variant, hipStream_t s, int *fits);
int mpg_cfu_auto(mpg_handle_s *h, hipStream_t s, int *cfu_variant);
int mpg_lfu_auto(mpg_handle_s *h, hipStream_t s, int *lf_variant);
int mpg_k_pole_fix(mpg_handle_s *h, const void *src, int src_type, int layout, int nlev, int nfields, void *dst, int dst_type,
                   double scale, double offset, hipStream_t s, const FieldTab &tab = FieldTab(), int64_t ld = 0);
int mpg_k_transpose_build(mpg_handle_s *h, hipStream_t s);
int mpg_k_transpose(mpg_handle_s *h, const void *src, int src_type, int64_t ld, int nlev, int nfields, void *dst, int dst_type, int layout,
                    hipStream_t s);
int mpg_k_apply_masked(mpg_handle_s *h, const void *src, int src_type, int layout, int nlev, int nfields, void *dst, int dst_type, int64_t ld,
                       const mpg_mask_opts *opts, hipStream_t s);
int mpg_k_store_to_mesh(mpg_grid_s *g, int stagger, mpg_mesh_s *m, int meshloc, int method, mpg_handle_s *h, hipStream_t s);
int mpg_k_store_periodic_to_mesh(mpg_grid_s *g, mpg_mesh_s *m, int meshloc, int pole_method, mpg_handle_s *h, hipStream_t s);
int mpg_k_grid_end_poles(mpg_grid_s *g, hipStream_t s);
int mpg_k_apply_to_mesh(mpg_handle_s *h, const void *src, int src_type, int64_t ld, int nlev, int nfields, void *dst, int dst_type, int layout,
                        double scale, double offset, hipStream_t s);
int mpg_k_wind_pair(bool edges, mpg_handle_s *hu, mpg_handle_s *hv, const double *c, const double *s_, const void *u, const void *v, int src_type,
                    int64_t ldu, int64_t ldv, int nlev, void *r0, void *r1, int dst_type, int layout, hipStream_t s);
int mpg_k_mesh_rotang(const mpg_grid_s *g, int64_t n, const double *x, const double *y, double *cosa, double *sina, hipStream_t s);
int mpg_k_mesh_edge_rotang(const mpg_grid_s *g, int64_t n, const double *x, const double *y, const double *angle, double *cn, double *sn,
                           hipStream_t s);
int mpg_k_store_conserve_to_mesh(mpg_grid_s *g, mpg_mesh_s *m, int norm_type, mpg_handle_s *h, hipStream_t s);
int mpg_k_conserve_rows(mpg_mesh_s *m, const int32_t *poff, const int32_t *pair_col, const double *pair_val, const int32_t *truncated, int cb,
                        int norm_type, const char *who, mpg_handle_s *h, hipStream_t s, const int32_t *extra_dev = nullptr,
                        int32_t *extra_host = nullptr, int nextra = 0);
int mpg_k_mesh_max_valence(mpg_mesh_s *m, hipStream_t s);
int mpg_k_store_conserve_mesh(mpg_mesh_s *src, mpg_mesh_s *dst, int norm_type, mpg_handle_s *h, hipStream_t s);
int mpg_k_apply_csr_rows(mpg_handle_s *h, const void *src, int src_type, int nlev, int nfields, void *dst, int dst_type, double scale,
                         double offset, hipStream_t s);
int mpg_k_apply_csr_to_mesh(mpg_handle_s *h, const void *src, int src_type, int64_t ld, int nlev, int nfields, void *dst, int dst_type, int layout,
                            double scale, double offset, hipStream_t s);
int mpg_k_nearest_points(mpg_mesh_s *m, const PointSet &pts, int64_t n, int32_t *idx, hipStream_t s);
int mpg_k_bvh_up(int64_t nchild, int64_t nparent, const double *child, double *parent, hipStream_t s);
int mpg_k_morton(int64_t n, const double *x, const double *y, const double *z, unsigned long long *key, int32_t *id, int64_t first, hipStream_t s);
int mpg_bvh_build(Bvh &b, int64_t n, const char *who, const std::function<int(unsigned long long *, int32_t *)> &keys,
                  const std::function<int()> &leaves, hipStream_t s, bool empty_leaf = false);
void mpg_bvh_view(const Bvh &b, BvhView &v);
int mpg_k_store_mesh(mpg_mesh_s *src, mpg_mesh_s *dst, int dst_meshloc, int method, mpg_handle_s *h, hipStream_t s);
int mpg_k_apply_rows(mpg_handle_s *h, const void *src, int src_type, int nlev, int nfields, void *dst, int dst_type, double scale, double offset,
                     hipStream_t s);
int mpg_k_bswap(void *buf, int64_t n, int elem_size, hipStream_t s);
int mpg_k_post_cast(const double *src, int64_t n, double scale, double offset, float *dst, int dst_be, hipStream_t s);
int mpg_k_post_layer_mean(const double *src, int nlevp1, int64_t P, float *dst, int dst_be, hipStream_t s);
int mpg_k_post_ptop(const double *src, int nlev, int64_t P, double *ptop_host, hipStream_t s);
int mpg_k_post_ptop_parts(const double *src, int nlev, int64_t P, double *vmax_host, double *candmin_host, int *has_cand_host, hipStream_t s);
int mpg_k_rotate(int64_t npts, int nlev, const double *cosa, const double *sina, double *u, double *v, hipStream_t s);
int mpg_k_wind_destagger(mpg_handle_s *h1, mpg_handle_s *h2, const double *cosa, const double *sina, const double *um, const double *vm, int nlev,
                         void *u, void *v, int dst_type, double *um_rot, double *vm_rot, hipStream_t s, int64_t ld = 0);
int mpg_k_pack(const double *src, int64_t n_src, int nlev, const int32_t *ids, int64_t n_ids, double *dst, hipStream_t s);
int mpg_k_tune(const char *key, int value);
int mpg_store_boxes();
int mpg_bilinear_linetype();
int mpg_node_fan_origin();
int mpg_grid_inside_tol_exp();
int mpg_nearest_variant();
void mpg_set_nearest_variant(int v);
int mpg_k_rebase(mpg_handle_s *h, int64_t base, int64_t n_local, hipStream_t s, bool keep_global = false);
int mpg_k_source_range(mpg_handle_s *h, int64_t *first, int64_t *end, hipStream_t s);
int mpg_k_unique_sources(mpg_handle_s *h, std::vector<int32_t> &ids, bool remap, hipStream_t s);
int mpg_scan_excl_i32(const int32_t *in, int32_t *out, int64_t n, hipStream_t s);
int mpg_sum_i32_i64(const int32_t *in, int64_t n, long long *out_dev, hipStream_t s);
int mpg_sort_pairs_u64_i32(const unsigned long long *keys_in, unsigned long long *keys_out, const int32_t *vals_in, int32_t *vals_out, int64_t n,
                           hipStream_t s);
```

Baseline: 2510.

## Consolidate conservative store status readbacks, fuse valence and scan totals into kernels

Several conservative-store setup changes are bundled. Status counters are merged into one device array so each stage does a single readback. Max valence is computed inside the raster kernel, the scan writes its last value and a 64-bit sum, and the clamp kernel and memsets are removed. Candidate storage moves to slot-major layout, and short CSR rows are sorted with a rank sort. Together these aim to cut host syncs, kernel launches and uncoalesced writes during weight-matrix construction. They likely matter little to the field-interpolation throughput metric unless setup is timed.

```diff
diff --git a/mpassit_amd/csrc/k_prims.hip b/mpassit_amd/csrc/k_prims.hip
--- a/mpassit_amd/csrc/k_prims.hip
+++ b/mpassit_amd/csrc/k_prims.hip
@@ -4,19 +4,35 @@
 #define SCAN_IPT 16
 #define SCAN_TILE (SCAN_NT * SCAN_IPT)
 
-__global__ __launch_bounds__(SCAN_NT) void k_scan_block_sums(const int32_t *__restrict__ in, int64_t n, int32_t *__restrict__ bsum) {
+template <bool SUM64>
+__global__ __launch_bounds__(SCAN_NT) void k_scan_block_sums(const int32_t *__restrict__ in, int64_t n, int32_t *__restrict__ bsum,
+                                                             unsigned long long *__restrict__ sum64) {
   __shared__ int32_t ws[SCAN_NT / 64];
+  __shared__ long long wl[SCAN_NT / 64];
   const int64_t base = (int64_t)blockIdx.x * SCAN_TILE;
   int32_t v = 0;
+  long long l = 0;
 #pragma unroll
   for (int k = 0; k < SCAN_IPT; ++k) {
     const int64_t i = base + (int64_t)k * SCAN_NT + threadIdx.x;
-    if (i < n) v += in[i];
+    if (i < n) {
+      const int32_t e = in[i];
+      v += e;
+      if (SUM64) l += e;
+    }
   }
   for (int o = 32; o > 0; o >>= 1) v += __shfl_down(v, o);
-  if ((threadIdx.x & 63) == 0) ws[threadIdx.x >> 6] = v;
+  if (SUM64)
+    for (int o = 32; o > 0; o >>= 1) l += __shfl_down(l, o);
+  if ((threadIdx.x & 63) == 0) {
+    ws[threadIdx.x >> 6] = v;
+    if (SUM64) wl[threadIdx.x >> 6] = l;
+  }
   __syncthreads();
-  if (threadIdx.x == 0) bsum[blockIdx.x] = ws[0] + ws[1] + ws[2] + ws[3];
+  if (threadIdx.x == 0) {
+    bsum[blockIdx.x] = ws[0] + ws[1] + ws[2] + ws[3];
+    if (SUM64) atomicAdd(sum64, (unsigned long long)(wl[0] + wl[1] + wl[2] + wl[3]));
+  }
 }
 
 __device__ __forceinline__ int32_t block_excl_scan(int32_t v, int32_t *total) {
@@ -48,7 +64,8 @@
   }
 }
 
-__global__ __launch_bounds__(SCAN_NT) void k_scan_apply(const int32_t *in, int64_t n, const int32_t *__restrict__ boff, int32_t *out) {
+__global__ __launch_bounds__(SCAN_NT) void k_scan_apply(const int32_t *in, int64_t n, const int32_t *__restrict__ boff, int32_t *out,
+                                                        int32_t *last) {
   const int64_t base = (int64_t)blockIdx.x * SCAN_TILE + (int64_t)threadIdx.x * SCAN_IPT;
   int32_t v[SCAN_IPT];
   int32_t sum = 0;
@@ -62,19 +79,21 @@
 #pragma unroll
   for (int k = 0; k < SCAN_IPT; ++k) {
     if (base + k < n) out[base + k] = run;
+    if (last && base + k == n - 1) *last = run;
     run += v[k];
   }
 }
 
-int mpg_scan_excl_i32(const int32_t *in, int32_t *out, int64_t n, hipStream_t s) {
+int mpg_scan_excl_i32(const int32_t *in, int32_t *out, int64_t n, hipStream_t s, int32_t *last_dev, long long *sum64_dev) {
   if (n <= 0) return MPG_SUCCESS;
   const int64_t nb = (n + SCAN_TILE - 1) / SCAN_TILE;
   TmpBuf<int32_t> bsum;
   int rc;
   if ((rc = bsum.alloc((size_t)nb, s))) return rc;
-  k_scan_block_sums<<<(unsigned)nb, SCAN_NT, 0, s>>>(in, n, bsum.p);
+  if (sum64_dev) k_scan_block_sums<true><<<(unsigned)nb, SCAN_NT, 0, s>>>(in, n, bsum.p, (unsigned long long *)sum64_dev);
+  else k_scan_block_sums<false><<<(unsigned)nb, SCAN_NT, 0, s>>>(in, n, bsum.p, nullptr);
   k_scan_sums<<<1, SCAN_NT, 0, s>>>(bsum.p, nb);
-  k_scan_apply<<<(unsigned)nb, SCAN_NT, 0, s>>>(in, n, bsum.p, out);
+  k_scan_apply<<<(unsigned)nb, SCAN_NT, 0, s>>>(in, n, bsum.p, out, last_dev);
   MPG_HIP(hipGetLastError());
   return MPG_SUCCESS;
 }
diff --git a/mpassit_amd/csrc/k_store_conserve.hip b/mpassit_amd/csrc/k_store_conserve.hip
--- a/mpassit_amd/csrc/k_store_conserve.hip
+++ b/mpassit_amd/csrc/k_store_conserve.hip
@@ -15,6 +15,10 @@
 #define CAND_CAP 24
 #define CONS_SPILL 256
 #define CONS_BIGBOX 128
+#ifndef CONS_SLOT_MAJOR
+#define CONS_SLOT_MAJOR 1
+#endif
+__device__ __forceinline__ int64_t cand_at(int64_t c, int e, int64_t nCells) { return CONS_SLOT_MAJOR ? (int64_t)e * nCells + c : c * CAND_CAP + e; }
 #define CONS_COOP_NT 64
 template <int MODE>
 __global__ __launch_bounds__(MODE == 3 ? 128 : CONS_COOP_NT) void k_conserve_raster(int64_t nCells, int maxEdges, const int32_t *__restrict__ voc,
@@ -26,7 +30,8 @@
                                                          int32_t *__restrict__ tmp_dst, int32_t *__restrict__ ovf, int32_t *__restrict__ n_ovf,
                                                          uint8_t *__restrict__ flip, const int32_t *__restrict__ poff,
                                                          int32_t *__restrict__ pair_c, int32_t *__restrict__ pair_p, const float *__restrict__ vij,
-                                                         float pad_coef, float pad_latlon, float e_max, int32_t *__restrict__ spill, int spill_cap) {
+                                                         float pad_coef, float pad_latlon, float e_max, int32_t *__restrict__ spill, int spill_cap,
+                                                         int count_valence) {
   constexpr bool COOP = MODE == 5 || MODE == 6;
   int64_t c = COOP ? (int64_t)ovf[blockIdx.x] : MODE == 7 ? (int64_t)pair_c[blockIdx.x] : blockIdx.x * (int64_t)blockDim.x + threadIdx.x;
   if (c >= nCells) return;
@@ -45,16 +50,31 @@
     }
   }
   int found = 0;
+  const int valence_seen = MODE == 3 && count_valence ? __hip_atomic_load(n_ovf + 1, __ATOMIC_RELAXED, __HIP_MEMORY_SCOPE_AGENT) : 0;
   dv3 poly[CONS_MAXV];
   int n = 0;
   for (int j = 0; j < maxEdges && n < CONS_MAXV; ++j) {
     int32_t v = voc[c * maxEdges + j];
     if (v > 0) poly[n++] = dv3{vx[v - 1], vy[v - 1], vz[v - 1]};
   }
-  if (n < 3) return;
+  if (MODE == 3 && count_valence) {
+    int mx = 0;
+#pragma unroll
+    for (int b = 8; b > 0; b >>= 1)
+      if (__ballot(n >= (mx | b))) mx |= b;
+    if (mx > valence_seen && (int)(threadIdx.x & 63) == __ffsll((long long)__ballot(1)) - 1) atomicMax(n_ovf + 1, mx);
+  }
+  if (MODE == 3 && c == nCells - 1) cnt_src[nCells] = 0;
+  if (n < 3) {
+    if (MODE == 3) { cnt_src[c] = 0; if (flip) flip[c] = 0; }
+    return;
+  }
   double area = 0.0;
   for (int i = 1; i + 1 < n; ++i) area += sph_tri_area(poly[0], poly[i], poly[i + 1]);
-  if (area == 0.0) return;
+  if (area == 0.0) {
+    if (MODE == 3) { cnt_src[c] = 0; if (flip) flip[c] = 0; }
+    return;
+  }
   if (MODE == 3 && flip) flip[c] = area < 0.0;
   if (area < 0.0)
     for (int i = 0; i < n / 2; ++i) {
@@ -160,13 +180,13 @@
             slot = __shfl(sl, 0);
             if (spill && slot < spill_cap) {
               __threadfence_block();
-              for (int k = lane; k < min(found, CAND_CAP); k += 64) spill[(int64_t)slot * CONS_SPILL + k] = tmp_dst[c * CAND_CAP + k];
+              for (int k = lane; k < min(found, CAND_CAP); k += 64) spill[(int64_t)slot * CONS_SPILL + k] = tmp_dst[cand_at(c, k, nCells)];
             } else {
               complete = false;
             }
           }
           if (is) {
-            if (pos < CAND_CAP) tmp_dst[c * CAND_CAP + pos] = pc;
+            if (pos < CAND_CAP) tmp_dst[cand_at(c, pos, nCells)] = pc;
             if (slot >= 0 && complete && pos < CONS_SPILL) spill[(int64_t)slot * CONS_SPILL + pos] = pc;
           }
           found += nnew;
@@ -182,13 +202,13 @@
           if (!candidate(i, j)) continue;
           const int32_t pc = (int32_t)((int64_t)j * nx + i);
           if (found < CAND_CAP) {
-            tmp_dst[c * CAND_CAP + found] = pc;
+            tmp_dst[cand_at(c, found, nCells)] = pc;
           } else {
             if (slot < 0) {
               slot = atomicAdd(n_ovf, 1);
               ovf[slot] = (int32_t)c;
               if (spill && slot < spill_cap)
-                for (int k = 0; k < CAND_CAP; ++k) spill[(int64_t)slot * CONS_SPILL + k] = tmp_dst[c * CAND_CAP + k];
+                for (int k = 0; k < CAND_CAP; ++k) spill[(int64_t)slot * CONS_SPILL + k] = tmp_dst[cand_at(c, k, nCells)];
               else
                 complete = false;
             }
@@ -269,7 +289,7 @@
               ovf[atomicAdd(n_ovf, 1)] = (int32_t)c;
               return;
             }
-            tmp_dst[c * CAND_CAP + found] = (int32_t)p;
+            tmp_dst[cand_at(c, found, nCells)] = (int32_t)p;
             ++found;
           } else if (MODE == 5) {
             const int slot = atomicAdd(&s_found, 1);
@@ -357,31 +377,53 @@
   return MPG_SUCCESS;
 }
 
+#define CSR_SORT_R 16
+template <int R>
+__device__ __forceinline__ void csr_rank_row(int b, int n, int32_t *__restrict__ col, double *__restrict__ val) {
+  int32_t kc[R];
+  double kv[R];
+#pragma unroll
+  for (int k = 0; k < R; ++k) {
+    kc[k] = k < n ? col[b + k] : INT32_MAX;
+    kv[k] = k < n ? val[b + k] : 0.0;
+  }
+#pragma unroll
+  for (int k = 0; k < R; ++k) {
+    int r = 0;
+#pragma unroll
+    for (int j = 0; j < R; ++j) r += kc[j] < kc[k];
+    if (k < n) {
+      col[b + r] = kc[k];
+      val[b + r] = kv[k];
+    }
+  }
+}
 __global__ __launch_bounds__(256) void k_csr_sort_rows(int64_t P, const int32_t *__restrict__ rowptr, int32_t *__restrict__ col,
                                                        double *__restrict__ val) {
   int64_t p = blockIdx.x * (int64_t)blockDim.x + threadIdx.x;
   if (p >= P) return;
   int b = rowptr[p], e = rowptr[p + 1];
-  for (int i = b + 1; i < e; ++i) {
-    int32_t kc = col[i];
-    double kv = val[i];
-    int j = i - 1;
-    while (j >= b && col[j] > kc) {
-      col[j + 1] = col[j];
-      val[j + 1] = val[j];
-      --j;
-    }
-    col[j + 1] = kc;
-    val[j + 1] = kv;
-  }
-}
-
-__global__ __launch_bounds__(256) void k_conserve_clamp_counts(int64_t nCells, const int32_t *__restrict__ cnt_src, int32_t *__restrict__ npair) {
-  int64_t c = blockIdx.x * (int64_t)blockDim.x + threadIdx.x;
-  if (c > nCells) return;
-  int n = c < nCells ? cnt_src[c] : 0;
-  npair[c] = n;
-}
+  const int n = e - b;
+  const bool wide = __any(n > CSR_SORT_R / 2 && n <= CSR_SORT_R);
+  if (n > CSR_SORT_R) {
+    for (int i = b + 1; i < e; ++i) {
+      int32_t kc = col[i];
+      double kv = val[i];
+      int j = i - 1;
+      while (j >= b && col[j] > kc) {
+        col[j + 1] = col[j];
+        val[j + 1] = val[j];
+        --j;
+      }
+      col[j + 1] = kc;
+      val[j + 1] = kv;
+    }
+  } else if (n > 1) {
+    if (wide) csr_rank_row<CSR_SORT_R>(b, n, col, val);
+    else csr_rank_row<CSR_SORT_R / 2>(b, n, col, val);
+  }
+}
+
 __global__ __launch_bounds__(256) void k_conserve_fill_pairs(int64_t nCells, const int32_t *__restrict__ npair, const int32_t *__restrict__ poff,
                                                              const int32_t *__restrict__ tmp_dst, int32_t *__restrict__ pair_c,
                                                              int32_t *__restrict__ pair_p) {
@@ -391,7 +433,7 @@
   if (n > CAND_CAP) return;
   for (int e = 0; e < n; ++e) {
     pair_c[o + e] = (int32_t)c;
-    pair_p[o + e] = tmp_dst[c * CAND_CAP + e];
+    pair_p[o + e] = tmp_dst[cand_at(c, e, nCells)];
   }
 }
 
@@ -486,31 +528,34 @@
 }
 
 struct ConsPairs {
-  TmpBuf<int32_t> count, cnt_src, tmp_dst, ovf, n_ovf, npair, poff, pair_c, pair_p, spill, bigq, truncated;
+  TmpBuf<int32_t> count, cnt_src, tmp_dst, ovf, status, poff, pair_c, pair_p, spill, bigq;
   TmpBuf<double> qarea, qsph, pair_val;
   TmpBuf<uint8_t> flip;
   TmpBuf<float> vij;
   int32_t npairs = 0, novf = 0, nbig = 0;
   int cb = 0;
 };
+static int read_status(const TmpBuf<int32_t> &status, int32_t *hs, hipStream_t s) {
+  MPG_HIP(hipMemcpyAsync(hs, status.p, CST_N * sizeof(int32_t), hipMemcpyDeviceToHost, s));
+  MPG_HIP(hipStreamSynchronize(s));
+  return MPG_SUCCESS;
+}
 static int conserve_pairs(mpg_mesh_s *m, mpg_grid_s *g, mpg_handle_s *h, hipStream_t s, bool raw, ConsPairs &X) {
   int rc;
   PointSet &cor = g->pts[MPG_STAGGERLOC_CORNER];
   const int nx = g->nx, ny = g->ny;
   const int64_t P = (int64_t)nx * ny;
-  TmpBuf<int32_t> &count = X.count, &cnt_src = X.cnt_src, &tmp_dst = X.tmp_dst, &ovf = X.ovf, &n_ovf = X.n_ovf, &npair = X.npair, &poff = X.poff,
+  TmpBuf<int32_t> &count = X.count, &cnt_src = X.cnt_src, &tmp_dst = X.tmp_dst, &ovf = X.ovf, &n_ovf = X.status, &poff = X.poff,
                   &pair_c = X.pair_c, &pair_p = X.pair_p;
   TmpBuf<double> &qarea = X.qarea, &qsph = X.qsph, &pair_val = X.pair_val;
   TmpBuf<uint8_t> &flip = X.flip;
   const int64_t nC = m->cwn;
   const double *vx = m->vx_g(), *vy = m->vy_g(), *vz = m->vz_g();
   if ((!raw && (rc = count.alloc((size_t)P + 1, s))) || (rc = qarea.alloc((size_t)P, s)) || (rc = qsph.alloc(4 * (size_t)P, s)) ||
-      (rc = cnt_src.alloc((size_t)nC, s)) || (rc = tmp_dst.alloc((size_t)nC * CAND_CAP, s)) || (rc = ovf.alloc((size_t)nC, s)) || (rc = n_ovf.alloc(5, s)) ||
-      (rc = npair.alloc((size_t)nC + 1, s)) || (rc = poff.alloc((size_t)nC + 1, s)) || (rc = flip.alloc((size_t)nC, s)))
+      (rc = cnt_src.alloc((size_t)nC + 1, s)) || (rc = tmp_dst.alloc((size_t)nC * CAND_CAP, s)) || (rc = ovf.alloc((size_t)nC, s)) ||
+      (rc = n_ovf.alloc(CST_N, s)) || (rc = poff.alloc((size_t)nC + 1, s)) || (rc = flip.alloc((size_t)nC, s)))
     return rc;
-  MPG_HIP(hipMemsetAsync(n_ovf.p, 0, 5 * sizeof(int32_t), s));
-  MPG_HIP(hipMemsetAsync(cnt_src.p, 0, sizeof(int32_t) * (size_t)nC, s));
-  MPG_HIP(hipMemsetAsync(flip.p, 0, (size_t)nC, s));
+  MPG_HIP(hipMemsetAsync(n_ovf.p, 0, CST_N * sizeof(int32_t), s));
   if (!raw) MPG_HIP(hipMemsetAsync(count.p, 0, sizeof(int32_t) * (P + 1), s));
   unsigned nb = (unsigned)((nC + 127) / 128);
   PyramidView pv = mpg_pyr_view(g->cellpyr);
@@ -526,67 +571,61 @@
   const int spill_cap = (int)std::min<int64_t>(nC, 1 << 16);
   TmpBuf<int32_t> &spill = X.spill, &bigq = X.bigq;
   if ((rc = spill.alloc((size_t)spill_cap * CONS_SPILL, s)) || (rc = bigq.alloc((size_t)spill_cap, s))) return rc;
+  const int count_valence = m->max_valence < 0;
   k_conserve_raster<3><<<nb, 128, 0, s>>>(nC, m->maxEdges, m->voc.p, vx, vy, vz, pv, nx, ny, cor.x.p, cor.y.p, cor.z.p,
                                         qarea.p, qsph.p, cnt_src.p, tmp_dst.p, ovf.p, n_ovf.p, flip.p, nullptr, vijp ? bigq.p : nullptr, nullptr, vijp,
-                                        (float)mpg_grid_box_pad_coef(g), (float)mpg_grid_box_pad_latlon(g), (float)mpg_grid_box_emax(g), spill.p, spill_cap);
-  if (m->max_valence < 0) k_max_valence<<<(unsigned)std::min<int64_t>((nC + 255) / 256, 2048), 256, 0, s>>>(nC, m->maxEdges, m->voc.p, n_ovf.p + 1);
+                                        (float)mpg_grid_box_pad_coef(g), (float)mpg_grid_box_pad_latlon(g), (float)mpg_grid_box_emax(g), spill.p, spill_cap,
+                                        count_valence);
   MPG_HIP(hipGetLastError());
-  int32_t &novf = X.novf, hv[3] = {0, 0, 0};
-  MPG_HIP(hipMemcpyAsync(hv, n_ovf.p, 3 * sizeof(int32_t), hipMemcpyDeviceToHost, s));
-  MPG_HIP(hipStreamSynchronize(s));
-  novf = hv[0];
-  if (m->max_valence < 0) m->max_valence = hv[1];
-  if (hv[2] > 0) {
-    k_conserve_raster<7><<<(unsigned)std::min(hv[2], spill_cap), 64, 0, s>>>(nC, m->maxEdges, m->voc.p, vx, vy, vz, pv, nx, ny, cor.x.p, cor.y.p, cor.z.p,
-                                                                            qarea.p, qsph.p, cnt_src.p, tmp_dst.p, ovf.p, n_ovf.p, nullptr, nullptr, bigq.p, nullptr,
-                                                                            vijp, (float)mpg_grid_box_pad_coef(g), (float)mpg_grid_box_pad_latlon(g),
-                                                                            (float)mpg_grid_box_emax(g), spill.p, spill_cap);
-    MPG_HIP(hipGetLastError());
-    MPG_HIP(hipMemcpyAsync(&novf, n_ovf.p, sizeof(int32_t), hipMemcpyDeviceToHost, s));
-    MPG_HIP(hipStreamSynchronize(s));
-  }
+  auto scan_pairs = [&]() -> int { return mpg_scan_excl_i32(cnt_src.p, poff.p, nC + 1, s, n_ovf.p + CST_NPAIR, (long long *)(n_ovf.p + CST_SUM64)); };
+  int32_t &novf = X.novf, hs[CST_N];
+  if ((rc = scan_pairs()) || (rc = read_status(n_ovf, hs, s))) return rc;
+  novf = hs[CST_OVF];
+  if (count_valence) m->max_valence = hs[CST_MAXV];
+  const int nbig = X.nbig = std::min(hs[CST_BIG], spill_cap);
   const unsigned coop_nt = CONS_COOP_NT;
-  if (novf > 0)
-    k_conserve_raster<5><<<(unsigned)novf, coop_nt, 0, s>>>(nC, m->maxEdges, m->voc.p, vx, vy, vz, pv, nx, ny, cor.x.p,
-                                                       cor.y.p, cor.z.p, qarea.p, qsph.p, cnt_src.p, nullptr, ovf.p, n_ovf.p, nullptr, nullptr,
-                                                       nullptr, nullptr, nullptr, 0.f, 0.f, 0.f, spill.p, spill_cap);
-  k_conserve_clamp_counts<<<(unsigned)((nC + 256) / 256), 256, 0, s>>>(nC, cnt_src.p, npair.p);
-  if ((rc = mpg_scan_excl_i32(npair.p, poff.p, nC + 1, s))) return rc;
+  if (nbig > 0 || novf > 0) {
+    if (nbig > 0) {
+      k_conserve_raster<7><<<(unsigned)nbig, 64, 0, s>>>(nC, m->maxEdges, m->voc.p, vx, vy, vz, pv, nx, ny, cor.x.p, cor.y.p, cor.z.p, qarea.p, qsph.p,
+                                                         cnt_src.p, tmp_dst.p, ovf.p, n_ovf.p, nullptr, nullptr, bigq.p, nullptr, vijp,
+                                                         (float)mpg_grid_box_pad_coef(g), (float)mpg_grid_box_pad_latlon(g),
+                                                         (float)mpg_grid_box_emax(g), spill.p, spill_cap, 0);
+      MPG_HIP(hipGetLastError());
+      if ((rc = read_status(n_ovf, hs, s))) return rc;
+      novf = hs[CST_OVF];
+    }
+    if (novf > 0)
+      k_conserve_raster<5><<<(unsigned)novf, coop_nt, 0, s>>>(nC, m->maxEdges, m->voc.p, vx, vy, vz, pv, nx, ny, cor.x.p,
+                                                         cor.y.p, cor.z.p, qarea.p, qsph.p, cnt_src.p, nullptr, ovf.p, n_ovf.p, nullptr, nullptr,
+                                                         nullptr, nullptr, nullptr, 0.f, 0.f, 0.f, spill.p, spill_cap, 0);
+    MPG_HIP(hipMemsetAsync(n_ovf.p + CST_SUM64, 0, sizeof(long long), s));
+    if ((rc = scan_pairs()) || (rc = read_status(n_ovf, hs, s))) return rc;
+  }
   int32_t &npairs = X.npairs;
-  long long total = 0;
-  {
-    TmpBuf<long long> tot;
-    if ((rc = tot.alloc(1, s))) return rc;
-    if ((rc = mpg_sum_i32_i64(npair.p, nC, tot.p, s))) return rc;
-    MPG_HIP(hipMemcpyAsync(&npairs, poff.p + nC, sizeof(int32_t), hipMemcpyDeviceToHost, s));
-    MPG_HIP(hipMemcpyAsync(&total, tot.p, sizeof(total), hipMemcpyDeviceToHost, s));
-    MPG_HIP(hipStreamSynchronize(s));
-    if (npairs < 0 || total != (long long)npairs) {
-      mpg_set_error("conservative RegridStore: %lld candidate pairs exceed 2^31", total);
-      return MPG_ERR_OVERFLOW;
-    }
+  npairs = hs[CST_NPAIR];
+  long long total;
+  memcpy(&total, hs + CST_SUM64, sizeof(total));
+  if (npairs < 0 || total != (long long)npairs) {
+    mpg_set_error("conservative RegridStore: %lld candidate pairs exceed 2^31", total);
+    return MPG_ERR_OVERFLOW;
   }
   if ((rc = pair_c.alloc((size_t)npairs + 1, s)) || (rc = pair_p.alloc((size_t)npairs + 1, s)) || (rc = pair_val.alloc((size_t)npairs + 1, s))) return rc;
-  k_conserve_fill_pairs<<<(unsigned)((nC + 255) / 256), 256, 0, s>>>(nC, npair.p, poff.p, tmp_dst.p, pair_c.p, pair_p.p);
+  k_conserve_fill_pairs<<<(unsigned)((nC + 255) / 256), 256, 0, s>>>(nC, cnt_src.p, poff.p, tmp_dst.p, pair_c.p, pair_p.p);
   if (novf > 0)
     k_conserve_raster<6><<<(unsigned)novf, coop_nt, 0, s>>>(nC, m->maxEdges, m->voc.p, vx, vy, vz, pv, nx, ny, cor.x.p,
                                                        cor.y.p, cor.z.p, qarea.p, qsph.p, nullptr, nullptr, ovf.p, n_ovf.p, nullptr, poff.p,
-                                                       pair_c.p, pair_p.p, nullptr, 0.f, 0.f, 0.f, spill.p, spill_cap);
+                                                       pair_c.p, pair_p.p, nullptr, 0.f, 0.f, 0.f, spill.p, spill_cap, 0);
   MPG_HIP(hipGetLastError());
   const int nv = std::max(3, std::min(m->max_valence, m->maxEdges));
   const int cb = X.cb = nv + 4 < CONS_BUF ? nv + 4 : CONS_BUF;
   const size_t clip_lds_bytes = sizeof(double) * cb * 3 * CLIP_NT;
   auto clip = raw ? k_conserve_clip_pairs<true> : k_conserve_clip_pairs<false>;
   if (clip_lds_bytes > 48 * 1024) MPG_HIP(hipFuncSetAttribute((const void *)clip, hipFuncAttributeMaxDynamicSharedMemorySize, (int)clip_lds_bytes));
-  TmpBuf<int32_t> &truncated = X.truncated;
-  if ((rc = truncated.alloc(1, s))) return rc;
-  MPG_HIP(hipMemsetAsync(truncated.p, 0, sizeof(int32_t), s));
   if (npairs > 0)
     clip<<<(unsigned)(((int64_t)npairs + CLIP_NT - 1) / CLIP_NT), CLIP_NT, clip_lds_bytes, s>>>(
         npairs, pair_c.p, pair_p.p, m->maxEdges, m->voc.p, vx, vy, vz, flip.p, nx, cor.x.p, cor.y.p, cor.z.p, qarea.p, cb,
-        pair_val.p, raw ? nullptr : count.p, truncated.p);
+        pair_val.p, raw ? nullptr : count.p, n_ovf.p + CST_TRUNC);
   MPG_HIP(hipGetLastError());
-  X.nbig = std::min(hv[2], spill_cap);
   return MPG_SUCCESS;
 }
 
@@ -621,17 +660,14 @@
   }
   ConsPairs X;
   if ((rc = h->rowptr.alloc((size_t)P + 1)) || (rc = conserve_pairs(m, g, h, s, false, X))) return rc;
-  TmpBuf<int32_t> &count = X.count, &n_ovf = X.n_ovf, &truncated = X.truncated, &pair_c = X.pair_c, &pair_p = X.pair_p;
+  TmpBuf<int32_t> &count = X.count, &pair_c = X.pair_c, &pair_p = X.pair_p;
   TmpBuf<double> &pair_val = X.pair_val;
   const int32_t npairs = X.npairs, novf = X.novf;
   const int cb = X.cb;
-  if ((rc = mpg_scan_excl_i32(count.p, h->rowptr.p, P + 1, s))) return rc;
-  int32_t nnz = 0, was_truncated = 0, hs[5] = {0, 0, 0, 0, 0};
-  MPG_HIP(hipMemcpyAsync(hs, n_ovf.p, sizeof(hs), hipMemcpyDeviceToHost, s));
-  MPG_HIP(hipMemcpyAsync(&nnz, h->rowptr.p + P, sizeof(int32_t), hipMemcpyDeviceToHost, s));
-  MPG_HIP(hipMemcpyAsync(&was_truncated, truncated.p, sizeof(int32_t), hipMemcpyDeviceToHost, s));
-  MPG_HIP(hipStreamSynchronize(s));
-  if (was_truncated) {
+  int32_t hs[CST_N];
+  if ((rc = mpg_scan_excl_i32(count.p, h->rowptr.p, P + 1, s, X.status.p + CST_NNZ)) || (rc = read_status(X.status, hs, s))) return rc;
+  const int32_t nnz = hs[CST_NNZ];
+  if (hs[CST_TRUNC]) {
     mpg_set_error("conservative RegridStore: a clipped polygon outgrew its %d vertex slots (a non-convex source cell?)", cb);
     return MPG_ERR_OVERFLOW;
   }
@@ -640,8 +676,8 @@
     return MPG_ERR_OVERFLOW;
   }
   h->nnz = nnz;
-  h->store_stats[1] = npairs; h->store_stats[2] = novf; h->store_stats[3] = X.nbig; h->store_stats[4] = hs[3];
-  h->store_stats[5] = hs[4]; h->store_stats[6] = cb;
+  h->store_stats[1] = npairs; h->store_stats[2] = novf; h->store_stats[3] = X.nbig; h->store_stats[4] = hs[CST_WALKED];
+  h->store_stats[5] = hs[CST_COPIED]; h->store_stats[6] = cb;
   if ((rc = h->col.alloc((size_t)nnz + 1)) || (rc = h->val.alloc((size_t)nnz + 1))) return rc;
   MPG_HIP(hipMemsetAsync(count.p, 0, sizeof(int32_t) * (P + 1), s));
   if (npairs > 0)
@@ -704,8 +740,8 @@
   for (int q = b; q < e; ++q) val[q] = val[q] / d;
 }
 
-int mpg_k_conserve_rows(mpg_mesh_s *m, const int32_t *poff, const int32_t *pair_col, const double *pair_val, const int32_t *truncated, int cb,
-                        int norm_type, const char *who, mpg_handle_s *h, hipStream_t s, const int32_t *extra_dev, int32_t *extra_host, int nextra) {
+int mpg_k_conserve_rows(mpg_mesh_s *m, const int32_t *poff, const int32_t *pair_col, const double *pair_val, int32_t *status, int cb,
+                        int norm_type, const char *who, mpg_handle_s *h, hipStream_t s, int32_t *status_host) {
   int rc;
   const int64_t nC = m->nCells;
   TmpBuf<double> carea;
@@ -714,13 +750,11 @@
   const double *vx = m->vx_g(), *vy = m->vy_g(), *vz = m->vz_g();
   k_conserve_tm_count<<<(unsigned)((nC + 256) / 256), 256, 0, s>>>(nC, m->maxEdges, m->voc.p, vx, vy, vz, poff, pair_val, carea.p, cnt.p);
   MPG_HIP(hipGetLastError());
-  if ((rc = mpg_scan_excl_i32(cnt.p, h->rowptr.p, nC + 1, s))) return rc;
-  int32_t nnz = 0, was_truncated = 0;
-  if (nextra > 0) MPG_HIP(hipMemcpyAsync(extra_host, extra_dev, sizeof(int32_t) * (size_t)nextra, hipMemcpyDeviceToHost, s));
-  MPG_HIP(hipMemcpyAsync(&nnz, h->rowptr.p + nC, sizeof(int32_t), hipMemcpyDeviceToHost, s));
-  MPG_HIP(hipMemcpyAsync(&was_truncated, truncated, sizeof(int32_t), hipMemcpyDeviceToHost, s));
+  if ((rc = mpg_scan_excl_i32(cnt.p, h->rowptr.p, nC + 1, s, status + CST_NNZ))) return rc;
+  MPG_HIP(hipMemcpyAsync(status_host, status, CST_N * sizeof(int32_t), hipMemcpyDeviceToHost, s));
   MPG_HIP(hipStreamSynchronize(s));
-  if (was_truncated) {
+  const int32_t nnz = status_host[CST_NNZ];
+  if (status_host[CST_TRUNC]) {
     mpg_set_error("%s: a clipped polygon outgrew its %d vertex slots (a non-convex mesh cell?)", who, cb);
     return MPG_ERR_OVERFLOW;
   }
@@ -768,11 +802,10 @@
   }
   ConsPairs X;
   if ((rc = conserve_pairs(m, g, h, s, true, X))) return rc;
-  int32_t hs[5] = {0, 0, 0, 0, 0};
-  if ((rc = mpg_k_conserve_rows(m, X.poff.p, X.pair_p.p, X.pair_val.p, X.truncated.p, X.cb, norm_type, "mpg_regrid_store_conserve_to_mesh", h, s, X.n_ovf.p, hs, 5)))
-    return rc;
-  h->store_stats[1] = X.npairs; h->store_stats[2] = X.novf; h->store_stats[3] = X.nbig; h->store_stats[4] = hs[3];
-  h->store_stats[5] = hs[4]; h->store_stats[6] = X.cb;
+  int32_t hs[CST_N];
+  if ((rc = mpg_k_conserve_rows(m, X.poff.p, X.pair_p.p, X.pair_val.p, X.status.p, X.cb, norm_type, "mpg_regrid_store_conserve_to_mesh", h, s, hs))) return rc;
+  h->store_stats[1] = X.npairs; h->store_stats[2] = X.novf; h->store_stats[3] = X.nbig; h->store_stats[4] = hs[CST_WALKED];
+  h->store_stats[5] = hs[CST_COPIED]; h->store_stats[6] = X.cb;
   return MPG_SUCCESS;
 }
 
diff --git a/mpassit_amd/csrc/k_store_conserve_mesh.hip b/mpassit_amd/csrc/k_store_conserve_mesh.hip
--- a/mpassit_amd/csrc/k_store_conserve_mesh.hip
+++ b/mpassit_amd/csrc/k_store_conserve_mesh.hip
@@ -274,11 +274,11 @@
     od = orient_d.p;
   }
   MPG_HIP(hipGetLastError());
-  TmpBuf<int32_t> cnt, poff, ovf, pair_d, pair_s, truncated;
+  TmpBuf<int32_t> cnt, poff, ovf, pair_d, pair_s, status;
   TmpBuf<double> pair_val;
-  if ((rc = cnt.alloc((size_t)nD + 1, s)) || (rc = poff.alloc((size_t)nD + 1, s)) || (rc = ovf.alloc(1, s)) || (rc = truncated.alloc(1, s))) return rc;
+  if ((rc = cnt.alloc((size_t)nD + 1, s)) || (rc = poff.alloc((size_t)nD + 1, s)) || (rc = ovf.alloc(1, s)) || (rc = status.alloc(CST_N, s))) return rc;
   MPG_HIP(hipMemsetAsync(ovf.p, 0, sizeof(int32_t), s));
-  MPG_HIP(hipMemsetAsync(truncated.p, 0, sizeof(int32_t), s));
+  MPG_HIP(hipMemsetAsync(status.p, 0, CST_N * sizeof(int32_t), s));
   const unsigned nbd = (unsigned)((nD + 256) / 256);
   k_cm_candidates<false><<<nbd, 256, 0, s>>>(nD, dst->maxEdges, dst->voc.p, dx, dy, dz, od, orient_s.p, v, cnt.p, nullptr, nullptr, nullptr, ovf.p);
   MPG_HIP(hipGetLastError());
@@ -313,9 +313,10 @@
   if (npairs > 0)
     k_cm_clip_pairs<<<(unsigned)(((int64_t)npairs + CLIP_NT - 1) / CLIP_NT), CLIP_NT, clip_lds_bytes, s>>>(
         npairs, pair_d.p, pair_s.p, src->maxEdges, src->voc.p, sx, sy, sz, orient_s.p, dst->maxEdges, dst->voc.p, dx, dy, dz, od, cb, pair_val.p,
-        truncated.p);
+        status.p + CST_TRUNC);
   MPG_HIP(hipGetLastError());
-  if ((rc = mpg_k_conserve_rows(dst, poff.p, pair_s.p, pair_val.p, truncated.p, cb, norm_type, "mpg_regrid_store_conserve_mesh", h, s))) return rc;
+  int32_t hs[CST_N];
+  if ((rc = mpg_k_conserve_rows(dst, poff.p, pair_s.p, pair_val.p, status.p, cb, norm_type, "mpg_regrid_store_conserve_mesh", h, s, hs))) return rc;
   h->store_stats[1] = npairs;
   h->store_stats[2] = 0;
   h->store_stats[3] = had ? 0 : (int64_t)(b.build_ms * 1e3f);
diff --git a/mpassit_amd/csrc/mpg_internal.h b/mpassit_amd/csrc/mpg_internal.h
--- a/mpassit_amd/csrc/mpg_internal.h
+++ b/mpassit_amd/csrc/mpg_internal.h
@@ -392,9 +392,9 @@
 int mpg_k_mesh_edge_rotang(const mpg_grid_s *g, int64_t n, const double *x, const double *y, const double *angle, double *cn, double *sn,
                            hipStream_t s);
 int mpg_k_store_conserve_to_mesh(mpg_grid_s *g, mpg_mesh_s *m, int norm_type, mpg_handle_s *h, hipStream_t s);
-int mpg_k_conserve_rows(mpg_mesh_s *m, const int32_t *poff, const int32_t *pair_col, const double *pair_val, const int32_t *truncated, int cb,
-                        int norm_type, const char *who, mpg_handle_s *h, hipStream_t s, const int32_t *extra_dev = nullptr,
-                        int32_t *extra_host = nullptr, int nextra = 0);
+enum { CST_OVF = 0, CST_MAXV = 1, CST_BIG = 2, CST_WALKED = 3, CST_COPIED = 4, CST_NPAIR = 5, CST_SUM64 = 6, CST_NNZ = 8, CST_TRUNC = 9, CST_N = 10 };
+int mpg_k_conserve_rows(mpg_mesh_s *m, const int32_t *poff, const int32_t *pair_col, const double *pair_val, int32_t *status, int cb,
+                        int norm_type, const char *who, mpg_handle_s *h, hipStream_t s, int32_t *status_host);
 int mpg_k_mesh_max_valence(mpg_mesh_s *m, hipStream_t s);
 int mpg_k_store_conserve_mesh(mpg_mesh_s *src, mpg_mesh_s *dst, int norm_type, mpg_handle_s *h, hipStream_t s);
 int mpg_k_apply_csr_rows(mpg_handle_s *h, const void *src, int src_type, int nlev, int nfields, void *dst, int dst_type, double scale,
@@ -429,7 +429,7 @@
 int mpg_k_rebase(mpg_handle_s *h, int64_t base, int64_t n_local, hipStream_t s, bool keep_global = false);
 int mpg_k_source_range(mpg_handle_s *h, int64_t *first, int64_t *end, hipStream_t s);
 int mpg_k_unique_sources(mpg_handle_s *h, std::vector<int32_t> &ids, bool remap, hipStream_t s);
-int mpg_scan_excl_i32(const int32_t *in, int32_t *out, int64_t n, hipStream_t s);
+int mpg_scan_excl_i32(const int32_t *in, int32_t *out, int64_t n, hipStream_t s, int32_t *last_dev = nullptr, long long *sum64_dev = nullptr);
 int mpg_sum_i32_i64(const int32_t *in, int64_t n, long long *out_dev, hipStream_t s);
 int mpg_sort_pairs_u64_i32(const unsigned long long *keys_in, unsigned long long *keys_out, const int32_t *vals_in, int32_t *vals_out, int64_t n,
                            hipStream_t s);
```

Result: no change. 2510, median of 4 (-0.0%).
